# iammadab/zk

Hardware: AMD Instinct MI355X
Metric: field-ops/sec (MLE fold, 2^24 evals, BN254 Fr) + sumcheck prover wall-clock (higher is better)
Workload: dtype u256 (8 x u32 Montgomery limbs, integer)

## Files before the change

### zk_amd/csrc/capi.hip

```cpp
#include <hip/hip_runtime.h>
#include <sched.h>

#include <algorithm>
#include <array>
#include <atomic>
#include <chrono>
#include <condition_variable>
#include <mutex>
#include <cstdio>
#include <map>
#include <new>
#include <set>
#include <string>
#include <thread>
#include <utility>
#include <vector>

#include "../../include/zk_amd.h"
#include "host_core.hpp"
#include "copy_helpers.hpp"
#include "prover_state.hpp"
#include "env.hpp"
#include "kernels.cuh"
#include "eval_kernels.cuh"
// ... 763 lines not shown
    uint32_t pos = tile_log;
    for (uint32_t p = 0; p < n_pass; ++p) {
        const uint32_t L = rem / n_pass + (p < rem % n_pass ? 1u : 0u);
        k_zeta_tile<<<(uint32_t)(1ull << (n_vars - kZetaTileLog)), kBlock, kZetaLdsBytes, c->stream>>>(t->d, pos, L, c->fi->P);
        HIPCHK(hipGetLastError());
        pos += L;
    }
    return ZK_OK;
}
static int32_t coeff_to_evaluation_device_sort(zk_ctx *c, uint64_t n_vars, const uint64_t *keys, const uint64_t *coeffs, uint64_t n_terms, zk_mle **out) {
    MleHolder t;
    ZKCHK(mle_alloc(c, n_vars, t.put()));
    size_t temp_bytes = 0;
    if (zeta_sort_terms(c->stream, nullptr, n_terms, (uint32_t)n_vars, nullptr, nullptr, nullptr, nullptr, nullptr, &temp_bytes) != 0) return ZK_ERR_HIP;
    const size_t w8 = (size_t)n_terms * 8, w4 = ((size_t)n_terms * 4 + 7) & ~(size_t)7;
    PoolBlock block;
    ZKCHK(block.alloc(c, 3 * w8 + 4 * w8 + 2 * w4 + ((temp_bytes + 255) & ~(size_t)255) + 256));
    DrainOnExit drain(c);
    uint8_t *blk = block.as<uint8_t>();
    uint64_t *d_keys = reinterpret_cast<uint64_t *>(blk), *d_idx_u = d_keys + n_terms, *d_idx_s = d_idx_u + n_terms, *d_coeffs = d_idx_s + n_terms;
    uint32_t *d_pos_u = reinterpret_cast<uint32_t *>(blk + 7 * w8), *d_perm = reinterpret_cast<uint32_t *>(blk + 7 * w8 + w4);
    void *temp = blk + 7 * w8 + 2 * w4;
    HIPCHK(hipMemcpyAsync(d_keys, keys, w8, hipMemcpyHostToDevice, c->stream));
    HIPCHK(hipMemcpyAsync(d_coeffs, coeffs, 4 * w8, hipMemcpyHostToDevice, c->stream));
    if (zeta_sort_terms(c->stream, d_keys, n_terms, (uint32_t)n_vars, d_idx_u, d_pos_u, d_idx_s, d_perm, temp, &temp_bytes) != 0) return ZK_ERR_HIP;
    ZKCHK(zeta_tiled_passes(c, t.get(), n_vars, d_idx_s, d_coeffs, n_terms, d_perm));
    ZKCHK(drain.wait());
    *out = t.release();
    return ZK_OK;
}
static int32_t coeff_to_evaluation_impl(zk_ctx *c, uint64_t n_vars, const uint64_t *keys, const uint64_t *coeffs, uint64_t n_terms,
                                        zk_mle **out) {
    if (!c || !out || (n_terms && (!keys || !coeffs))) return ZK_ERR_BAD_ARG;
    if (n_vars == 0 || n_vars > kMaxVars) return ZK_ERR_EVAL_LEN;
    for (uint64_t t = 0; t < n_terms; ++t)
        if (keys[t] >> n_vars) return ZK_ERR_COEFF_RANGE;
    ZKCHK(use_device(c));
    static const bool global_passes_flag = env_flag("ZK_ZETA_GLOBAL");
    if (!global_passes_flag && n_terms && n_terms >= zeta_device_sort_min() && n_terms < ((uint64_t)1 << 32))
        return coeff_to_evaluation_device_sort(c, n_vars, keys, coeffs, n_terms, out);
    std::vector<std::pair<uint64_t, uint64_t>> order(n_terms);
    for (uint64_t t = 0; t < n_terms; ++t) order[t] = {bit_reverse64(keys[t]) >> (64 - n_vars), t};
    std::sort(order.begin(), order.end());
    const size_t stage_bytes = (size_t)n_terms * 40;
    std::vector<uint64_t> pageable;
    uint64_t *hs = nullptr;
    if (stage_bytes <= ((size_t)1 << 20)) {
        uint8_t *blk = nullptr;
        ZKCHK(results_staging(c, stage_bytes ? stage_bytes : 8, &blk));
        hs = reinterpret_cast<uint64_t *>(blk);
    } else {
        pageable.resize((size_t)n_terms * 5);
        hs = pageable.data();
    }
    uint64_t m = 0;
    {
        uint64_t *hk = hs, *hc = hs + n_terms;
        for (uint64_t i = 0; i < n_terms;) {
            Fe acc = fe_from_u64limbs(coeffs + 4 * order[i].second);
            uint64_t j = i + 1;
            for (; j < n_terms && order[j].first == order[i].first; ++j)
                acc = fe_add(acc, fe_from_u64limbs(coeffs + 4 * order[j].second), c->fi->P);
            hk[m] = order[i].first;
            fe_to_u64limbs(acc, hc + 4 * m);
            ++m;
            i = j;
        }
    }
    MleHolder t;
    ZKCHK(mle_alloc(c, n_vars, t.put()));
    PoolBlock terms;
    uint64_t *d_keys = nullptr, *d_coeffs = nullptr;
    if (m) ZKCHK(terms.alloc(c, stage_bytes));
    DrainOnExit drain(c);
    if (m) {
        HIPCHK(hipMemcpyAsync(terms.p, hs, (size_t)(n_terms + 4 * m) * 8, hipMemcpyHostToDevice, c->stream));
        d_keys = terms.as();
        d_coeffs = d_keys + n_terms;
    }
    static const bool global_passes = env_flag("ZK_ZETA_GLOBAL");
    if (!global_passes) {
        ZKCHK(zeta_tiled_passes(c, t.get(), n_vars, d_keys, d_coeffs, m, nullptr));
    } else {
        HIPCHK(hipMemsetAsync(t->d, 0, (size_t)32 << n_vars, c->stream));
        if (m) {
            k_scatter_terms<<<grid_for(m), kBlock, 0, c->stream>>>(d_keys, d_coeffs, m, t->d);
            HIPCHK(hipGetLastError());
        }
        for (uint32_t b = 0; b < n_vars;) {
            const uint32_t v = n_vars - b >= 3 ? 3u : (uint32_t)(n_vars - b);
            const uint64_t groups = 1ull << (n_vars - v);
            uint64_t g = (groups + kBlock - 1) / kBlock;
            if (g > kMaxGridStream) g = kMaxGridStream;
            if (v == 3) k_zeta_multi<3><<<(uint32_t)g, kBlock, 0, c->stream>>>(t->d, groups, b, c->fi->P);
            else if (v == 2) k_zeta_multi<2><<<(uint32_t)g, kBlock, 0, c->stream>>>(t->d, groups, b, c->fi->P);
            else k_zeta_pass<<<(uint32_t)g, kBlock, 0, c->stream>>>(t->d, groups, b, c->fi->P);
            HIPCHK(hipGetLastError());
            b += v;
        }
    }
    ZKCHK(drain.wait());
    *out = t.release();
    return ZK_OK;
}
extern "C" int32_t zk_coeff_to_evaluation(zk_ctx *c, uint64_t n_vars, const uint64_t *keys, const uint64_t *coeffs, uint64_t n_terms,
                                          zk_mle **out) {
    try {
        return coeff_to_evaluation_impl(c, n_vars, keys, coeffs, n_terms, out);
    } catch (const std::bad_alloc &) {
        return ZK_ERR_ALLOC;
    } catch (...) {
        return ZK_ERR_BAD_ARG;
    }
}

extern "C" int32_t zk_product_check(const zk_mle *const *f, uint64_t k) {
    if (k == 0) return ZK_ERR_EMPTY_PRODUCT;
    if (!f) return ZK_ERR_BAD_ARG;
    for (uint64_t i = 0; i < k; ++i) {
        if (!f[i]) return ZK_ERR_BAD_ARG;
        if (f[i]->n_vars != f[0]->n_vars) return ZK_ERR_ARITY_MISMATCH;
        if (f[i]->ctx != f[0]->ctx) return ZK_ERR_CONTEXT_MISMATCH;
    }
    return ZK_OK;
}
static int32_t product_args(zk_ctx *c, const zk_mle *const *f, uint64_t k) {
    if (!c) return ZK_ERR_BAD_ARG;
    ZKCHK(zk_product_check(f, k));
    if (f[0]->ctx != c) return ZK_ERR_CONTEXT_MISMATCH;
    if (k > (uint64_t)kMaxFactors) return ZK_ERR_UNSUPPORTED;
    return use_device(c);
}

extern "C" int32_t zk_prod_reduce(zk_ctx *c, const zk_mle *const *f, uint64_t k, zk_mle **out) {
    if (!out) return ZK_ERR_BAD_ARG;
    ZKCHK(product_args(c, f, k));
    zk_mle *o = nullptr;
    ZKCHK(mle_alloc(c, f[0]->n_vars, &o));
    FactorPtrs fp = {};
    for (uint64_t i = 0; i < k; ++i) fp.in[i] = f[i]->d;
    const uint64_t n = 1ull << f[0]->n_vars;
    if (n >= 64) {
        uint64_t g = n / kBlock;
        if (g > 2 * kMaxGridStream) g = 2 * kMaxGridStream;
        k_prod_reduce_run<<<(uint32_t)(g ? g : 1), kBlock, 0, c->stream>>>(fp, (int)k, n, o->d, c->fi->P);
    } else {
        k_prod_reduce<<<grid_for(n), kBlock, 0, c->stream>>>(fp, (int)k, n, o->d, c->fi->P);
    }
    HIPCHK(hipGetLastError());
    *out = o;
    return ZK_OK;
}

extern "C" int32_t zk_product_evaluate(zk_ctx *c, const zk_mle *const *f, uint64_t k, const uint64_t *point,
                                       uint64_t n_point, uint64_t out[4]) {
    if (!out || (!point && n_point)) return ZK_ERR_BAD_ARG;
    ZKCHK(product_args(c, f, k));
    if (n_point != f[0]->n_vars) return ZK_ERR_EVAL_ARITY;
    Fe prod = fe_one(c->fi->P);
    for (uint64_t i = 0; i < k; ++i) {
        uint64_t v[4];
        ZKCHK(zk_mle_evaluate(c, f[i], point, n_point, v));
        prod = fe_mul(prod, fe_from_u64limbs(v), c->fi->P);
    }
    fe_to_u64limbs(prod, out);
    return ZK_OK;
}

static inline uint64_t *epart_counters(uint64_t *d_epart) { return d_epart + 2 * (kEpartBytes / 8); }
static int32_t scratch_alloc(zk_ctx *c, ProverScratch &ps, uint64_t rounds, uint32_t D, const DeviceChain *chain = nullptr) {
    ps = ProverScratch{};
    ps.rp_bytes = (size_t)(rounds ? rounds : 1) * (D + 1) * 32;
    ps.ch_bytes = (size_t)(rounds ? rounds : 1) * 32;
    if (chain) {
        ps.external = true;
        ps.d_sponge = chain->d_sponge;
        ps.d_rp = chain->d_rp;
        ps.d_ch = chain->d_ch;
        ps.d_final = chain->d_final;
        ps.d_epart = chain->d_epart;
    } else {
        ZKCHK(ps.sponge_block.alloc(c, sizeof(WordSponge)));
        ps.d_sponge = ps.sponge_block.as<WordSponge>();
    }
    ZKCHK(ps.chal_block.alloc(c, kChalBlockBytes));
    ps.d_challenge = ps.chal_block.as();
    ps.d_claim = ps.d_challenge + 2 * kChalWords;
    if (chain) return ZK_OK;
    ZKCHK(ps.epart_block.alloc(c, kEpartBlockBytes));
    ps.d_epart = ps.epart_block.as();
    ZKCHK(ps.proof_block.alloc(c, ps.proof_block_bytes()));
    ps.d_rp = ps.proof_block.as();
    ps.d_ch = ps.d_rp + ps.rp_bytes / 8;
    ps.d_final = ps.d_ch + ps.ch_bytes / 8;
    return ZK_OK;
}
int32_t zk::results_staging(zk_ctx *c, size_t bytes, uint8_t **out) {
    if (c->h_results_bytes < bytes) {
        if (c->h_results) (void)hipHostFree(c->h_results);
        c->h_results = nullptr;
        c->h_results_bytes = 0;
        size_t cap = 1 << 16;
        while (cap < bytes) cap <<= 1;
        HIPCHK(hipHostMalloc((void **)&c->h_results, cap, kPolledHostFlags));
        c->h_results_bytes = cap;
    }
    *out = c->h_results;
    return ZK_OK;
}

static inline uint64_t partials_capacity() { return g_batch ? (uint64_t)kMaxGrid * kMaxSums / kMaxBatch : (uint64_t)kMaxGrid * kMaxSums; }
static inline uint64_t *partials_of(zk_ctx *c) { return g_batch ? c->d_partials + (size_t)g_batch->cur * partials_capacity() * 4 : c->d_partials; }
static inline RoundLaunchCtx launch_ctx(zk_ctx *c) {
    RoundLaunchCtx lc = {c->stream, &c->fi->P, partials_of(c), partials_capacity(), {}};
    return lc;
}
static int32_t launch_tail(zk_ctx *c, uint32_t nblocks, uint32_t ns, WordSponge *sponge, uint64_t *out_rp, uint64_t *out_ch, uint64_t *d_challenge,
                           uint64_t *lanes, const TailDerive &dv, const PendingSponge *init = nullptr) {
    const uint64_t *part = partials_of(c);
    hipStream_t st = c->stream;
    const FieldParams *P = &c->fi->P;
    if (init && init->valid && sponge == init->dst && !lanes && !g_batch) {
        k_round_tail_init<<<1, kBlock, 0, st>>>(part, nblocks, ns, sponge, out_rp, out_ch, d_challenge, *P, dv, init->w, init->zero2);
        HIPCHK(hipGetLastError());
        return ZK_OK;
    }
    if (init && init->valid) {
        k_store_sponge<<<1, 64, 0, st>>>(init->w, init->dst, init->zero2);
        HIPCHK(hipGetLastError());
    }
    auto single = [=]() {
        k_round_tail<<<1, kBlock, 0, st>>>(part, nblocks, ns, sponge, out_rp, out_ch, d_challenge, lanes, *P, dv);
        return hipGetLastError();
    };
    if (!lanes && batch_record(BK_TAIL, 0, 1, kBlock, 0, nblocks, ns, 0, 0, TailSlot{part, sponge, out_rp, out_ch, d_challenge, dv}, single)) return ZK_OK;
    HIPCHK(single());
    return ZK_OK;
}
int32_t zk::launch_reduce_tail(zk_ctx *c, uint32_t nblocks, uint32_t ns, uint64_t *out_rp) {
    k_round_tail<<<1, kBlock, 0, c->stream>>>(c->d_partials, nblocks, ns, nullptr, out_rp, nullptr, nullptr, nullptr, c->fi->P);
    HIPCHK(hipGetLastError());
    return ZK_OK;
}
static bool claim_in_round() {
    static const bool v = env_u64("ZK_CLAIM_IN_ROUND", 1, 0, 1) != 0;
    return v;
}
static inline bool fast_degree(uint32_t D) { return D >= 1 && D <= 4; }

struct TailTargets {
    WordSponge *sponge;
    uint64_t *out_rp;
    uint64_t *out_ch;
    uint64_t *d_challenge;
    uint64_t *lanes;
    const PendingSponge *init;
    uint64_t *claim_park;
    TailDerive *lanes_dv;
};
static std::vector<Fe> interp_weights_compute(uint32_t D, const FieldParams &P) {
    std::vector<Fe> w(D + 1);
    for (uint32_t i = 0; i <= D; ++i) {
        Fe den = fe_one(P);
        const Fe xi = fe_from_u32(i, P);
        for (uint32_t j = 0; j <= D; ++j)
            if (j != i) den = fe_mul(den, fe_sub(xi, fe_from_u32(j, P), P), P);
        w[i] = fe_inverse(den, P);
    }
    return w;
}
static std::vector<Fe> interp_weights(uint32_t D, const FieldParams &P) {
    static std::mutex mu;
    static std::map<std::pair<std::array<uint32_t, 8>, uint32_t>, std::vector<Fe>> cache;
    std::array<uint32_t, 8> key;
    for (int i = 0; i < 8; ++i) key[i] = P.p[i];
    std::lock_guard<std::mutex> lock(mu);
    auto it = cache.find({key, D});
    if (it == cache.end()) it = cache.emplace(std::make_pair(key, D), interp_weights_compute(D, P)).first;
    return it->second;
}
static uint64_t skip1_min_pairs() {
    static const uint64_t v = env_u64("ZK_SKIP1_MIN_PAIRS", (uint64_t)1 << 16, 1, (uint64_t)1 << 40);
    return v;
}
static inline TermSpec single_term(int k) {
    TermSpec ts = {1, {k, 0, 0, 0}};
    return ts;
}
struct DeferredTail {
    uint32_t blocks;
    bool skip1;
    bool lead;
    const uint64_t *claim;
};
static uint64_t lead_min_pairs() {
    static const uint64_t v = env_u64("ZK_LEAD_MIN_PAIRS", (uint64_t)1 << 16, 1, (uint64_t)1 << 40);
    return v;
}
static bool shard_skip_on() {
    static const bool v = env_u64("ZK_SHARD_SKIP1", 1, 0, 1) != 0;
    return v;
}
static int32_t launch_sums(zk_ctx *c, const FactorPtrs &fp, const TermSpec &ts, uint64_t q, uint32_t D, bool fused,
                           const uint64_t *d_r, const TailTargets &tt, const TailDerive *dv = nullptr, DeferredTail *defer = nullptr) {
    if (defer) defer->blocks = 0;
    const FieldParams &P = c->fi->P;
    if (fast_degree(D)) {
        uint32_t total = 0;
        int first = 0;
        const bool may_derive = !tt.lanes || (tt.lanes_dv && shard_skip_on());
        bool skip1 = dv && dv->prev_rp && tt.claim_park && fused && may_derive && D <= (uint32_t)kMaxSkipDegree && q >= skip1_min_pairs();
        bool lead = may_derive && q >= lead_min_pairs();
        ClaimJob cjob = {};
        if (skip1 && claim_in_round()) cjob = ClaimJob{dv->prev_rp, dv->prev_chal, dv->w, tt.claim_park, D + 1};
        auto with_claim = [&](RoundLaunchCtx lc) {
            lc.claim = cjob;
            return lc;
        };
        auto tail_dv = [&]() {
            TailDerive t = skip1 && dv ? *dv : TailDerive{};
            t.lead = lead ? D : 0;
            t.claim = (t.prev_rp && cjob.out) ? cjob.out : nullptr;
            if (tt.lanes) {
                if (tt.lanes_dv) *tt.lanes_dv = t;
                t.local_only = 1;
            }
            return t;
        };
        if (tt.lanes_dv) *tt.lanes_dv = TailDerive{};
        if (ts.n_terms == 2 && ts.term_k[1] == 1) {
            uint32_t g = 0;
            const int lrc = launch_round_plus1(with_claim(launch_ctx(c)), fp, ts.term_k[0], q, D, fused, d_r, &g, &skip1, &lead);
            if (lrc == kLaunchHipError) {
                g_hip_err = "round kernel launch failed";
                return ZK_ERR_HIP;
            }
            if (lrc == kLaunchOk) {
                if (defer) {
                    defer->blocks = g;
                    defer->skip1 = skip1;
                    defer->claim = skip1 ? cjob.out : nullptr;
                    defer->lead = lead;
                    return ZK_OK;
                }
                return launch_tail(c, g, D + 1, tt.sponge, tt.out_rp, tt.out_ch, tt.d_challenge, tt.lanes, tail_dv(), tt.init);
            }
        }
        if (ts.n_terms != 1) {
            skip1 = lead = false;
            cjob = {};
        }
        for (int i = 0; i < ts.n_terms; ++i) {
            FactorPtrs sub = {};
            for (int f = 0; f < ts.term_k[i]; ++f) {
                sub.in[f] = fp.in[first + f];
                sub.out[f] = fp.out[first + f];
            }
            RoundLaunchCtx lc = with_claim(launch_ctx(c));
            lc.d_partials += (size_t)total * (D + 1) * 4;
            lc.capacity_elems -= (uint64_t)total * (D + 1);
            uint32_t g = 0;
            const int lrc = launch_round(lc, sub, ts.term_k[i], q, D, fused, d_r, &g, &skip1, &lead);
            if (lrc == kLaunchUnsupported) return ZK_ERR_UNSUPPORTED;
            if (lrc != kLaunchOk) {
                g_hip_err = "round kernel launch failed";
                return ZK_ERR_HIP;
            }
            total += g;
            first += ts.term_k[i];
        }
        if (defer) {
            defer->blocks = total;
            defer->skip1 = skip1;
            defer->claim = skip1 ? cjob.out : nullptr;
            defer->lead = lead;
            return ZK_OK;
        }
        return launch_tail(c, total, D + 1, tt.sponge, tt.out_rp, tt.out_ch, tt.d_challenge, tt.lanes, tail_dv(), tt.init);
    }
    if (ts.n_terms != 1) return ZK_ERR_UNSUPPORTED;
    const int k = ts.term_k[0];
    for (uint32_t t = 0; t <= D; ++t) {
        uint32_t g = 0;
        if (launch_round_single_t(launch_ctx(c), fp, k, q, fe_from_u32(t, P), &g) != kLaunchOk) {
            g_hip_err = "round kernel launch failed";
            return ZK_ERR_HIP;
        }
        k_round_tail<<<1, kBlock, 0, c->stream>>>(c->d_partials, g, 1, nullptr, c->d_sums + 4 * t, nullptr, nullptr, nullptr, P);
        HIPCHK(hipGetLastError());
    }
    k_round_tail<<<1, kBlock, 0, c->stream>>>(c->d_sums, 1, D + 1, tt.sponge, tt.out_rp, tt.out_ch, tt.d_challenge, tt.lanes, P);
    HIPCHK(hipGetLastError());
    return ZK_OK;
}

extern "C" int32_t zk_round_sums(zk_ctx *c, const zk_mle *const *f, uint64_t k, uint32_t D, uint64_t *out) {
    if (!out) return ZK_ERR_BAD_ARG;
    ZKCHK(product_args(c, f, k));
    if (D >= kMaxSums) return ZK_ERR_UNSUPPORTED;
    if (f[0]->n_vars == 0) return ZK_ERR_PANIC_INDEX;
    FactorPtrs fp = {};
    for (uint64_t i = 0; i < k; ++i) fp.in[i] = f[i]->d;
    const uint64_t q = 1ull << (f[0]->n_vars - 1);
    uint64_t *d_out = c->d_sums + 4 * kMaxSums;
    TailTargets tt = {nullptr, d_out, nullptr, nullptr, nullptr, nullptr, nullptr};
    ZKCHK(launch_sums(c, fp, single_term((int)k), q, D, false, nullptr, tt));
    HIPCHK(hipMemcpyAsync(out, d_out, (size_t)(D + 1) * 32, hipMemcpyDeviceToHost, c->stream));
    HIPCHK(hipStreamSynchronize(c->stream));
    return ZK_OK;
}

extern "C" int32_t zk_transcript_new(zk_transcript **out) {
    if (!out) return ZK_ERR_BAD_ARG;
    zk_transcript *t = new (std::nothrow) zk_transcript();
    if (!t) return ZK_ERR_ALLOC;
    t->sp.init();
    *out = t;
    return ZK_OK;
}
extern "C" int32_t zk_transcript_free(zk_transcript *t) {
    delete t;
    return ZK_OK;
}
extern "C" int32_t zk_transcript_append(zk_transcript *t, const uint8_t *data, size_t len) {
    if (!t || (!data && len)) return ZK_ERR_BAD_ARG;
    t->sp.update(data, len);
    return ZK_OK;
}
extern "C" int32_t zk_transcript_sample_challenge(zk_transcript *t, uint8_t out[32]) {
    if (!t || !out) return ZK_ERR_BAD_ARG;
    t->sp.sample_challenge(out);
    return ZK_OK;
}
extern "C" int32_t zk_transcript_sample_field_element(zk_transcript *t, int32_t field, uint64_t out[4]) {
    if (!t || !out) return ZK_ERR_BAD_ARG;
    const FieldInfo *fi = field_info(field);
    if (!fi) return ZK_ERR_BAD_FIELD;
    uint8_t h[32];
    t->sp.sample_challenge(h);
    fe_to_u64limbs(fe_from_be_bytes_mod_order(h, 32, fi->P), out);
    return ZK_OK;
}
extern "C" int32_t zk_transcript_sample_n_field_elements(zk_transcript *t, int32_t field, uint64_t n, uint64_t *out) {
    if (!t || (!out && n)) return ZK_ERR_BAD_ARG;
    if (!field_info(field)) return ZK_ERR_BAD_FIELD;
    for (uint64_t i = 0; i < n; ++i) ZKCHK(zk_transcript_sample_field_element(t, field, out + 4 * i));
    return ZK_OK;
}
extern "C" int32_t zk_keccak256(const uint8_t *data, size_t len, uint8_t out[32]) {
    if ((!data && len) || !out) return ZK_ERR_BAD_ARG;
    Sponge s;
    s.init();
    s.update(data, len);
    s.finalize_reset(out);
    return ZK_OK;
}

void zk::absorb_elements(Sponge &sp, const uint64_t *elems, uint64_t n, const FieldParams &P) {
    uint8_t b[32];
    for (uint64_t i = 0; i < n; ++i) {
        fe_to_bytes_be(fe_from_u64limbs(elems + 4 * i), P, b);
        sp.update(b, 32);
    }
}
Fe zk::squeeze_field_element(Sponge &sp, const FieldParams &P) {
    uint8_t h[32];
    sp.sample_challenge(h);
    return fe_from_be_bytes_mod_order(h, 32, P);
}
int32_t zk::host_staging(zk_ctx *c, size_t cb) {
    if (c->h_absorb_bytes < cb) {
        for (int b = 0; b < 2; ++b) {
            if (c->h_absorb[b]) (void)hipHostFree(c->h_absorb[b]);
            c->h_absorb[b] = nullptr;
        }
        c->h_absorb_bytes = 0;
        for (int b = 0; b < 2; ++b) HIPCHK(hipHostMalloc((void **)&c->h_absorb[b], cb, hipHostMallocDefault));
        c->h_absorb_bytes = cb;
    }
    if (!c->ev_absorb[0])
        for (int b = 0; b < 2; ++b) HIPCHK(hipEventCreateWithFlags(&c->ev_absorb[b], hipEventDisableTiming));
    return ZK_OK;
}
int32_t zk::stream_table_bytes(zk_ctx *c, const zk_mle *const *f, uint64_t k, const std::function<void(const uint8_t *, size_t)> &consume) {
    const uint64_t n = 1ull << f[0]->n_vars;
    const uint64_t chunk = n < (1ull << 19) ? n : (1ull << 19);
    const size_t cb = (size_t)chunk * 32;
    const uint64_t per_table = n / chunk, total = per_table * k;
    ZKCHK(host_staging(c, cb));
    PoolBlock d_bytes[2];
    ZKCHK(d_bytes[0].alloc(c, cb));
    ZKCHK(d_bytes[1].alloc(c, cb));
    DrainOnExit drain(c);
    auto enqueue = [&](uint64_t i) -> int32_t {
        const int b = (int)(i & 1);
        const uint64_t *src = f[i / per_table]->d + 4 * (i % per_table) * chunk;
        k_to_bytes<<<grid_for(chunk), kBlock, 0, c->stream>>>(src, d_bytes[b].as<uint8_t>(), chunk, c->fi->P);
        HIPCHK(hipGetLastError());
        HIPCHK(hipMemcpyAsync(c->h_absorb[b], d_bytes[b].p, cb, hipMemcpyDeviceToHost, c->stream));
        HIPCHK(hipEventRecord(c->ev_absorb[b], c->stream));
        return ZK_OK;
    };
    ZKCHK(enqueue(0));
    for (uint64_t i = 0; i < total; ++i) {
        if (i + 1 < total) ZKCHK(enqueue(i + 1));
        HIPCHK(hipEventSynchronize(c->ev_absorb[i & 1]));
        consume(c->h_absorb[i & 1], cb);
    }
    drain.armed = false;
    return ZK_OK;
}
static int32_t absorb_tables(zk_ctx *c, Sponge &sp, zk_mle *const *f, uint64_t k) {
    return stream_table_bytes(c, (const zk_mle *const *)f, k, [&](const uint8_t *p, size_t bytes) { sp.update(p, bytes); });
}

static inline uint64_t *chal_of_round(const RoundState &st, uint64_t round) { return st.ps.d_challenge + (round & 1) * kChalWords; }
static inline uint64_t *chal_cur(const RoundState &st) { return chal_of_round(st, st.round); }
static inline uint64_t *chal_prev(const RoundState &st) { return chal_of_round(st, st.round + 1); }
static inline uint64_t *epart_of_round(const RoundState &st, uint64_t round) { return st.ps.d_epart + (round & 1) * (kEpartBytes / 8); }
static inline uint32_t *epart_counter(const RoundState &st, uint64_t round) {
    return reinterpret_cast<uint32_t *>(st.ps.d_epart + 2 * (kEpartBytes / 8) + (round & 1));
}
static int32_t round_state_init(RoundState &st, zk_ctx *c, zk_mle *const *f, uint64_t k, uint32_t D, bool consume,
                                uint64_t total_rounds, const DeviceChain *chain = nullptr) {
    st.c = c;
    st.k = k;
    st.vars_left = f[0]->n_vars;
    st.round = 0;
    st.D = D;
    st.pending_fold = false;
    st.first_out_of_place = !consume;
    st.terms = single_term((int)k);
    st.d_final = nullptr;
    st.dv = {};
    st.pipe_active = false;
    st.pipe_blocks = 0;
    st.pipe_total = true;
    st.pub = {};
    st.published = false;
    st.init.valid = false;
    for (uint64_t i = 0; i < (uint64_t)kMaxFactors; ++i) {
        st.cur[i] = i < k ? f[i]->d : nullptr;
        st.scratch[i].reset();
    }
    ZKCHK(scratch_alloc(c, st.ps, total_rounds, D, chain));
    if (D >= 1 && D <= (uint32_t)kMaxSkipDegree) {
        auto it = c->lagrange_w.find(D);
        if (it == c->lagrange_w.end()) {
            const std::vector<Fe> w = interp_weights(D, c->fi->P);
            std::vector<uint64_t> limbs(4 * (size_t)(D + 1));
            for (uint32_t t = 0; t <= D; ++t) fe_to_u64limbs(w[t], limbs.data() + 4 * t);
            RawBlock d_w;
            ZKCHK(raw_alloc(c, limbs.size() * 8, d_w.put()));
            HIPCHK(hipMemcpy(d_w.get(), limbs.data(), limbs.size() * 8, hipMemcpyHostToDevice));
            it = c->lagrange_w.emplace(D, static_cast<uint64_t *>(d_w.release())).first;
        }
        st.dv.w = it->second;
    }
    if (!consume && st.vars_left >= 2)
        for (uint64_t i = 0; i < k; ++i) ZKCHK(st.scratch[i].alloc(c, (size_t)32 << (st.vars_left - 1)));
    return ZK_OK;
}
static int32_t flush_pending_sponge(RoundState &st) {
    if (!st.init.valid) return ZK_OK;
    st.init.valid = false;
    k_store_sponge<<<1, 64, 0, st.c->stream>>>(st.init.w, st.init.dst, st.init.zero2);
    HIPCHK(hipGetLastError());
    return ZK_OK;
}
static int32_t round_enqueue(RoundState &st, uint64_t *lanes, DeferredTail *defer = nullptr, TailDerive *lanes_dv = nullptr) {
    zk_ctx *c = st.c;
    if (st.pending_fold) st.vars_left -= 1;
    const uint64_t m = st.vars_left;
    if (m == 0) return ZK_ERR_BAD_ARG;
    const uint64_t q = 1ull << (m - 1);
    FactorPtrs fp = {};
    for (uint64_t i = 0; i < st.k; ++i) {
        fp.in[i] = st.cur[i];
        fp.out[i] = (st.pending_fold && st.first_out_of_place && st.scratch[i]) ? st.scratch[i].as() : st.cur[i];
    }
    TailTargets tt;
    tt.sponge = lanes ? nullptr : st.ps.d_sponge;
    tt.out_rp = st.ps.d_rp + st.round * (st.D + 1) * 4;
    tt.out_ch = st.ps.d_ch + st.round * 4;
    tt.d_challenge = chal_cur(st);
    tt.lanes = lanes;
    tt.claim_park = st.ps.d_claim;
    tt.lanes_dv = lanes_dv;
    tt.init = nullptr;
    if (st.init.valid) {
        if (!lanes && !defer && fast_degree(st.D) && !st.pending_fold) tt.init = &st.init;
        else ZKCHK(flush_pending_sponge(st));
    }
    int32_t rc;
    if (st.pending_fold && !fast_degree(st.D)) {
        Fe r;
        (void)r;
        for (uint64_t i = 0; i < st.k; ++i) {
            k_fold_dev<<<grid_for(q * 2), kBlock, 0, c->stream>>>(fp.in[i], fp.out[i], q * 2, (uint32_t)m, c->fi->P, chal_prev(st));
            HIPCHK(hipGetLastError());
        }
        FactorPtrs g = {};
        for (uint64_t i = 0; i < st.k; ++i) g.in[i] = fp.out[i];
        rc = launch_sums(c, g, st.terms, q, st.D, false, nullptr, tt);
    } else {
        st.dv.prev_rp = st.round ? tt.out_rp - (size_t)(st.D + 1) * 4 : nullptr;
        st.dv.prev_chal = chal_prev(st);
        rc = launch_sums(c, fp, st.terms, q, st.D, st.pending_fold, chal_prev(st), tt, &st.dv, defer);
        if (tt.init) st.init.valid = false;
    }
    if (st.pending_fold) {
        for (uint64_t i = 0; i < st.k; ++i) st.cur[i] = fp.out[i];
        st.first_out_of_place = false;
    }
    st.pending_fold = true;
    return rc;
}

static uint64_t pipe_max_pairs() {
    static const uint64_t v = [] {
        uint64_t x = env_u64("ZK_PIPE_MAX_PAIRS", (uint64_t)1 << 12, 0, (uint64_t)1 << 40);
        const uint64_t cap = (uint64_t)kPipeMaxWorkBlocks * 16 * kMaxLazy;
        return x > cap ? cap : x;
    }();
    return v;
}
static inline uint64_t pipe_limit_pairs() { return pipe_max_pairs(); }
static bool pipe_shape(const RoundState &st, int *k, int *extra) {
    if (st.terms.n_terms == 1) {
        *k = st.terms.term_k[0];
        *extra = 0;
    } else if (st.terms.n_terms == 2 && st.terms.term_k[1] == 1) {
        *k = st.terms.term_k[0];
        *extra = 1;
    } else {
        return false;
    }
    return pipe_shape_ok(*k, st.D, *extra);
}
static constexpr size_t kDbgWords = 64 * 32 + 64 * 16;
static uint64_t *pipe_dbg_slot(zk_ctx *c, bool finisher) {
    static const bool on = env_flag("ZK_PIPE_DEBUG");
    if (!on) return nullptr;
    if (!c->d_dbg) {
        if (hipMalloc(&c->d_dbg, kDbgWords * 8) != hipSuccess) return nullptr;
        (void)hipMemset(c->d_dbg, 0, kDbgWords * 8);
    }
    if (finisher) return c->d_dbg + 64 * 32;
    const uint32_t i = c->dbg_launch++ % 64;
    return c->d_dbg + (size_t)i * 32;
}
static void pipe_dbg_dump(zk_ctx *c) {
    if (!c->d_dbg) return;
    std::vector<uint64_t> h(kDbgWords);
    if (hipMemcpy(h.data(), c->d_dbg, kDbgWords * 8, hipMemcpyDeviceToHost) != hipSuccess) return;
    uint64_t t0 = 0;
    for (uint32_t i = 0; i < c->dbg_launch && i < 64; ++i) {
        const uint64_t *d = h.data() + (size_t)i * 32;
        if (!t0) t0 = d[0];
        fprintf(stderr, "[pipe %2u] tail: start %7.2f red %5.2f eval %5.2f transcript %5.2f publish %5.2f | work: start %7.2f loop %5.2f close %5.2f store %5.2f\n", i,
                (d[0] - t0) / 100.0, (d[1] - d[0]) / 100.0, (d[2] - d[1]) / 100.0, (d[3] - d[2]) / 100.0, (d[4] - d[3]) / 100.0,
                d[8] ? (d[8] - t0) / 100.0 : 0.0, (d[9] - d[8]) / 100.0, (d[10] - d[9]) / 100.0, (d[11] - d[10]) / 100.0);
    }
    const uint64_t *f = h.data() + 64 * 32;
    for (uint32_t r = 0; r < 24 && f[16 * r]; ++r) {
        const uint64_t *d = f + 16 * r;
        fprintf(stderr, "[fin %2u] start %7.2f gather %5.2f eval %5.2f transcript %5.2f barrier %5.2f | work %5.2f (from %5.2f)\n", r, (d[0] - t0) / 100.0,
                (d[1] - d[0]) / 100.0, (d[2] - d[1]) / 100.0, (d[3] - d[2]) / 100.0, (d[4] - d[3]) / 100.0, d[8] ? (d[9] - d[8]) / 100.0 : 0.0,
                d[8] ? (d[8] - d[0]) / 100.0 : 0.0);
    }
    (void)hipMemset(c->d_dbg, 0, kDbgWords * 8);
    c->dbg_launch = 0;
}
static bool finish_pipe_on() {
    static const bool v = env_u64("ZK_FINISH_PIPE", 1, 0, 1) != 0;
    return v;
}
static bool finish_pipe_applies(const RoundState &st) {
    int k, extra;
    if (!finish_pipe_on() || !pipe_shape(st, &k, &extra)) return false;
    return st.vars_left >= 3 && st.vars_left - 1 <= (uint64_t)finish_pipe_max_vars(k + extra);
}
static bool pipe_wants_next(const RoundState &st, uint64_t m_s) {
    int k, extra;
    if (!pipe_limit_pairs() || !pipe_shape(st, &k, &extra)) return false;
    if (m_s < 3) return false;
    if (!finish_pipe_on() && m_s - 1 <= (uint64_t)kFinishVars) return false;
    return ((uint64_t)1 << (m_s - 2)) <= pipe_limit_pairs();
}
static int32_t finish_pipe_enqueue(RoundState &st) {
    zk_ctx *c = st.c;
    int k = 0, extra = 0;
    (void)pipe_shape(st, &k, &extra);
    FinishPipeLaunch fl = {};
    fl.k = k;
    fl.extra = extra;
    fl.D = st.D;
    fl.m_in = (uint32_t)st.vars_left;
    fl.entry = st.pipe_active ? 2 : (st.pending_fold ? 1 : 0);
    fl.e_partials = epart_of_round(st, st.round);
    fl.e_blocks = 1;
    if (st.pipe_active && !st.pipe_total) {
        fl.e_partials += (size_t)pipe_values_per_block(k, st.D) * 4;
        fl.e_blocks = st.pipe_blocks;
    }
    fl.pc = c->pipe_consts;
    fl.chal_in = chal_prev(st);
    const uint64_t remaining = st.pending_fold ? st.vars_left - 1 : st.vars_left;
    fl.chal_last = chal_of_round(st, st.round + remaining - 1);
    fl.sponge = st.ps.d_sponge;
    fl.out_rp = st.ps.d_rp + st.round * (st.D + 1) * 4;
    fl.out_ch = st.ps.d_ch + st.round * 4;
    fl.out_final = st.d_final;
    fl.dbg = pipe_dbg_slot(c, true);
    fl.pub = st.pub;
    FactorPtrs fp = {};
    for (uint64_t i = 0; i < st.k; ++i) fp.in[i] = st.cur[i];
    const int lrc = launch_finish_pipe(launch_ctx(c), fp, fl);
    if (lrc != kLaunchOk) {
        g_hip_err = "pipelined finisher launch failed";
        return lrc == kLaunchUnsupported ? ZK_ERR_UNSUPPORTED : ZK_ERR_HIP;
    }
    st.round += remaining;
    st.vars_left = 0;
    st.pending_fold = false;
    st.pipe_active = false;
    st.published = st.pub.flag != nullptr;
    return ZK_OK;
}
static PipeTailArgs pipe_tail_args(const RoundState &st, int mode, const uint64_t *partials, uint32_t nblocks, uint32_t n_in) {
    PipeTailArgs ta = {};
    ta.dbg = pipe_dbg_slot(st.c, false);
    ta.partials = partials;
    ta.nblocks = nblocks;
    ta.n_in = n_in;
    ta.mode = mode;
    ta.chal_in = chal_prev(st);
    ta.chal_out = chal_cur(st);
    ta.sponge = st.ps.d_sponge;
    ta.out_rp = st.ps.d_rp + st.round * (st.D + 1) * 4;
    ta.out_ch = st.ps.d_ch + st.round * 4;
    ta.pc = st.c->pipe_consts;
    return ta;
}
static int32_t pipe_enter(RoundState &st, const DeferredTail &dt) {
    zk_ctx *c = st.c;
    int k = 0, extra = 0;
    (void)pipe_shape(st, &k, &extra);
    PipeLaunch pl = {};
    pl.k = k;
    pl.extra = extra;
    pl.D = st.D;
    pl.fold = false;
    pl.emit = 1;
    pl.q = (uint64_t)1 << (st.vars_left - 2);
    pl.chal_fold = nullptr;
    pl.e_partials = epart_of_round(st, st.round + 1);
    pl.done_counter = epart_counter(st, st.round + 1);
    pl.tail = pipe_tail_args(st, 0, partials_of(c), dt.blocks, st.D + 1);
    if (dt.skip1) {
        pl.tail.dv = st.dv;
        pl.tail.dv.prev_rp = pl.tail.out_rp - (size_t)(st.D + 1) * 4;
        pl.tail.dv.prev_chal = chal_prev(st);
        pl.tail.dv.claim = dt.claim;
    }
    pl.tail.dv.lead = dt.lead ? st.D : 0;
    FactorPtrs fp = {};
    for (uint64_t i = 0; i < st.k; ++i) fp.in[i] = fp.out[i] = st.cur[i];
    uint32_t g = 0;
    const int lrc = launch_round_pipe(launch_ctx(c), fp, pl, &g);
    if (lrc != kLaunchOk) {
        g_hip_err = "pipelined round launch failed";
        return lrc == kLaunchUnsupported ? ZK_ERR_UNSUPPORTED : ZK_ERR_HIP;
    }
    st.pipe_active = true;
    st.pipe_blocks = g;
    st.pipe_total = true;
    return ZK_OK;
}
static int32_t pipe_step(RoundState &st) {
    zk_ctx *c = st.c;
    int k = 0, extra = 0;
    (void)pipe_shape(st, &k, &extra);
    const uint64_t m = st.vars_left;
    const bool stay = pipe_wants_next(st, m - 1);
    PipeLaunch pl = {};
    pl.k = k;
    pl.extra = extra;
    pl.D = st.D;
    pl.fold = true;
    pl.emit = stay ? 1 : 0;
    pl.q = m >= 3 ? (uint64_t)1 << (m - 3) : 0;
    if (pl.q == 0) return ZK_ERR_BAD_ARG;
    pl.chal_fold = chal_prev(st);
    pl.e_partials = epart_of_round(st, st.round + 1);
    pl.done_counter = epart_counter(st, st.round + 1);
    pl.tail = pipe_tail_args(st, 1, epart_of_round(st, st.round), 1, pipe_values_per_block(k, st.D));
    if (!st.pipe_total) {
        pl.tail.partials = epart_of_round(st, st.round) + (size_t)pipe_values_per_block(k, st.D) * 4;
        pl.tail.nblocks = st.pipe_blocks;
    }
    FactorPtrs fp = {};
    for (uint64_t i = 0; i < st.k; ++i) {
        fp.in[i] = st.cur[i];
        fp.out[i] = (st.first_out_of_place && st.scratch[i]) ? st.scratch[i].as() : st.cur[i];
    }
    uint32_t g = 0;
    const int lrc = launch_round_pipe(launch_ctx(c), fp, pl, &g);
    if (lrc != kLaunchOk) {
        g_hip_err = "pipelined round launch failed";
        return lrc == kLaunchUnsupported ? ZK_ERR_UNSUPPORTED : ZK_ERR_HIP;
    }
    for (uint64_t i = 0; i < st.k; ++i) st.cur[i] = fp.out[i];
    st.first_out_of_place = false;
    st.vars_left = m - 1;
    st.pipe_active = stay;
    st.pipe_blocks = g;
    st.pipe_total = true;
    ++st.round;
    return ZK_OK;
}

template <int K, int D>
static int32_t launch_finish(zk_ctx *c, const FactorPtrs &fp, uint32_t m_in, int pending, uint64_t *d_challenge, WordSponge *sp,
                             uint64_t *out_rp, uint64_t *out_ch, uint64_t *out_final) {
    const uint32_t m = pending ? m_in - 1 : m_in;
    const size_t lds = (size_t)K * ((size_t)32 << m) + (kBlock / 64) * (D + 1) * 32 + (D + 1) * 32 + 48;
    HIPCHK(hipFuncSetAttribute(reinterpret_cast<const void *>(&k_finish<K, D>), hipFuncAttributeMaxDynamicSharedMemorySize, (int)lds));
    hipStream_t st = c->stream;
    const FieldParams *P = &c->fi->P;
    auto single = [=]() {
        k_finish<K, D><<<1, kBlock, lds, st>>>(fp, m_in, pending, *P, d_challenge, sp, out_rp, out_ch, out_final);
        return hipGetLastError();
    };
    if (batch_record_other(single)) return ZK_OK;
    HIPCHK(single());
    return ZK_OK;
}
static bool finish_shape_ok(uint64_t k, uint32_t D) {
    const int shape = (int)k * 10 + (int)D;
    return shape == 11 || shape == 12 || shape == 21 || shape == 22 || shape == 23 || shape == 32 || shape == 33;
}
static int32_t finish_enqueue(RoundState &st) {
    zk_ctx *c = st.c;
    FactorPtrs fp = {};
    for (uint64_t i = 0; i < st.k; ++i) fp.in[i] = st.cur[i];
    const int pending = st.pending_fold ? 1 : 0;
    const uint32_t m_in = (uint32_t)st.vars_left;
    const uint64_t remaining = pending ? st.vars_left - 1 : st.vars_left;
    uint64_t *out_rp = st.ps.d_rp + st.round * (st.D + 1) * 4, *out_ch = st.ps.d_ch + st.round * 4;
    int32_t rc = ZK_ERR_UNSUPPORTED;
    if (st.terms.n_terms > 1) {
        const uint32_t m = pending ? m_in - 1 : m_in;
        const size_t lds = (size_t)st.k * ((size_t)32 << m) + (kBlock / 64) * (st.D + 1) * 32 + (st.D + 1) * 32 + 48;
        const FieldParams &P = c->fi->P;
#define ZK_FINISH_TERMS(DD)                                                                                                     \
    case DD:                                                                                                                    \
        if (hipFuncSetAttribute(reinterpret_cast<const void *>(&k_finish_terms<DD>), hipFuncAttributeMaxDynamicSharedMemorySize, \
                                (int)lds) != hipSuccess)                                                                        \
            return ZK_ERR_HIP;                                                                                                  \
        k_finish_terms<DD><<<1, kBlock, lds, c->stream>>>(fp, st.terms, m_in, pending, P, chal_prev(st), st.ps.d_sponge,     \
                                                          out_rp, out_ch, st.d_final);                                          \
        break;
        switch (st.D) {
            ZK_FINISH_TERMS(1)
            ZK_FINISH_TERMS(2)
            ZK_FINISH_TERMS(3)
            ZK_FINISH_TERMS(4)
            default: return ZK_ERR_UNSUPPORTED;
        }
#undef ZK_FINISH_TERMS
        rc = hipGetLastError() == hipSuccess ? ZK_OK : ZK_ERR_HIP;
    } else {
        switch ((int)st.k * 10 + (int)st.D) {
            case 11: rc = launch_finish<1, 1>(c, fp, m_in, pending, chal_prev(st), st.ps.d_sponge, out_rp, out_ch, st.d_final); break;
            case 12: rc = launch_finish<1, 2>(c, fp, m_in, pending, chal_prev(st), st.ps.d_sponge, out_rp, out_ch, st.d_final); break;
            case 21: rc = launch_finish<2, 1>(c, fp, m_in, pending, chal_prev(st), st.ps.d_sponge, out_rp, out_ch, st.d_final); break;
            case 22: rc = launch_finish<2, 2>(c, fp, m_in, pending, chal_prev(st), st.ps.d_sponge, out_rp, out_ch, st.d_final); break;
            case 23: rc = launch_finish<2, 3>(c, fp, m_in, pending, chal_prev(st), st.ps.d_sponge, out_rp, out_ch, st.d_final); break;
            case 32: rc = launch_finish<3, 2>(c, fp, m_in, pending, chal_prev(st), st.ps.d_sponge, out_rp, out_ch, st.d_final); break;
            case 33: rc = launch_finish<3, 3>(c, fp, m_in, pending, chal_prev(st), st.ps.d_sponge, out_rp, out_ch, st.d_final); break;
            default: break;
        }
    }
    if (rc == ZK_OK) {
        st.round += remaining;
        st.vars_left = 0;
        st.pending_fold = false;
    }
    return rc;
}
static inline bool finish_applies(const RoundState &st) {
    if (st.terms.n_terms == 1 ? !finish_shape_ok(st.k, st.D) : !fast_degree(st.D)) return false;
    const uint64_t after = st.pending_fold ? st.vars_left - 1 : st.vars_left;
    return after >= 1 && after <= (uint64_t)kFinishVars;
}

static int32_t prover_step(RoundState &st, bool *finished_in_kernel) {
    if (st.init.valid && (finish_pipe_applies(st) || st.pipe_active || finish_applies(st))) ZKCHK(flush_pending_sponge(st));
    if (finish_pipe_applies(st)) {
        *finished_in_kernel = true;
        return finish_pipe_enqueue(st);
    }
    if (st.pipe_active) return pipe_step(st);
    if (finish_applies(st)) {
        *finished_in_kernel = true;
        return finish_enqueue(st);
    }
    const uint64_t m_s = st.pending_fold ? st.vars_left - 1 : st.vars_left;
    DeferredTail dt = {0, false, false, nullptr};
    const bool enter = fast_degree(st.D) && pipe_wants_next(st, m_s);
// ... 752 lines not shown
```

### zk_amd/csrc/launch.hpp

```cpp
#pragma once
#include <hip/hip_runtime.h>
#include <stdint.h>

#include <cstring>
#include <functional>
#include <type_traits>
#include <vector>

#include "common.cuh"

namespace zk {

enum BatchKernel : int { BK_STORE_SPONGE = 1, BK_ROUND_KD, BK_ROUND0_DOT29, BK_ROUND_QUAD, BK_TAIL, BK_PIPE, BK_FINISH_PIPE, BK_OTHER };
struct BatchRecord {
    int kernel;
    uint32_t shape;
    uint32_t grid, block;
    size_t lds;
    uint64_t s[4];
    std::function<hipError_t()> single;
    alignas(16) unsigned char slot[384];
};
struct BatchRecorder {
    int n = 0;
    int cur = 0;
    hipStream_t stream = nullptr;
    const FieldParams *P = nullptr;
    std::vector<BatchRecord> recs[kMaxBatch];
    uint64_t merged = 0, replayed = 0;
};
extern thread_local BatchRecorder *g_batch;
template <class Slot, class F>
inline bool batch_record(int kernel, uint32_t shape, uint32_t grid, uint32_t block, size_t lds, uint64_t s0, uint64_t s1, uint64_t s2, uint64_t s3,
                         const Slot &slot, F &&single) {
    BatchRecorder *r = g_batch;
    if (!r) return false;
    static_assert(sizeof(Slot) <= sizeof(BatchRecord::slot), "slot does not fit a batch record");
    static_assert(std::is_trivially_copyable<Slot>::value, "slots are plain data");
    r->recs[r->cur].emplace_back();
    BatchRecord &rec = r->recs[r->cur].back();
    rec.kernel = kernel;
    rec.shape = shape;
    rec.grid = grid;
    rec.block = block;
    rec.lds = lds;
    rec.s[0] = s0, rec.s[1] = s1, rec.s[2] = s2, rec.s[3] = s3;
    rec.single = std::function<hipError_t()>(std::forward<F>(single));
    std::memcpy(rec.slot, &slot, sizeof(Slot));
    return true;
}
template <class F>
inline bool batch_record_other(F &&single) {
    struct Nothing {
        int x;
    } none = {0};
    return batch_record(BK_OTHER, 0, 0, 0, 0, 0, 0, 0, 0, none, std::forward<F>(single));
}
int batch_launch_rounds(const BatchRecorder &r, size_t idx);
int batch_launch_pipe(const BatchRecorder &r, size_t idx);
template <class Slot>
inline void batch_gather(const BatchRecorder &r, size_t idx, BatchOf<Slot> &out) {
    std::memset(&out, 0, sizeof out);
    for (int b = 0; b < r.n; ++b) std::memcpy(&out.a[b], r.recs[b][idx].slot, sizeof(Slot));
}

struct RoundLaunchCtx {
    hipStream_t stream;
    const FieldParams *P;
    uint64_t *d_partials;
    uint64_t capacity_elems;
    ClaimJob claim;
};
enum { kLaunchOk = 0, kLaunchUnsupported = -1, kLaunchHipError = -2 };
int launch_round(const RoundLaunchCtx &lc, const FactorPtrs &fp, int k, uint64_t q, uint32_t D, bool fused,
                 const uint64_t *d_r, uint32_t *out_grid, bool *skip1 = nullptr, bool *lead = nullptr);
int launch_round_plus1(const RoundLaunchCtx &lc, const FactorPtrs &fp, int k, uint64_t q, uint32_t D, bool fused,
                       const uint64_t *d_r, uint32_t *out_grid, bool *skip1 = nullptr, bool *lead = nullptr);
int launch_round_single_t(const RoundLaunchCtx &lc, const FactorPtrs &fp, int k, uint64_t q, const Fe &tval, uint32_t *out_grid);


constexpr uint32_t kPipeMaxWorkBlocks = 256;
}
#include "pipe_args.hpp"
namespace zk {
struct PipeLaunch {
    int k, extra;
    uint32_t D;
    bool fold;
    int emit;
    uint64_t q;
    const uint64_t *chal_fold;
    uint64_t *e_partials;
    uint32_t *done_counter;
    PipeTailArgs tail;
};
bool pipe_shape_ok(int k, uint32_t D, int extra);
uint32_t pipe_values_per_block(int k, uint32_t D);
uint32_t pipe_rows_per_block(int k, uint32_t D, int extra);
uint32_t pipe_work_blocks(int k, uint32_t D, int extra, uint64_t q);
int launch_round_pipe(const RoundLaunchCtx &lc, const FactorPtrs &fp, const PipeLaunch &pl, uint32_t *out_work_blocks);
int launch_spin_us(hipStream_t stream, uint32_t us);
struct FinishPipeLaunch {
    int k, extra;
    uint32_t D;
    uint32_t m_in;
    int entry;
    const uint64_t *e_partials;
    uint32_t e_blocks;
    PipeConsts pc;
    const uint64_t *chal_in;
    uint64_t *chal_last;
    WordSponge *sponge;
    uint64_t *out_rp, *out_ch, *out_final;
    uint64_t *dbg;
    FinishPublish pub;
};
int launch_finish_pipe(const RoundLaunchCtx &lc, const FactorPtrs &fp, const FinishPipeLaunch &fl);
uint32_t finish_pipe_max_vars(int n_factors);

}
```

### zk_amd/csrc/prover_state.hpp

```cpp
#pragma once
#include "host_core.hpp"

constexpr size_t kChalWords = kChallengeBytes / 8;
constexpr size_t kEpartBytes = (size_t)(kPipeMaxWorkBlocks + 2) * 16 * 32;
constexpr size_t kChalBlockBytes = 2 * kChallengeBytes + 32;
constexpr size_t kEpartBlockBytes = 2 * kEpartBytes + 16;
struct ProverScratch {
    WordSponge *d_sponge;
    uint64_t *d_challenge;
    uint64_t *d_claim;
    uint64_t *d_epart;
    uint64_t *d_rp;
    uint64_t *d_ch;
    uint64_t *d_final;
    size_t rp_bytes, ch_bytes;
    bool external;
    PoolBlock sponge_block, chal_block, epart_block, proof_block;
    size_t proof_block_bytes() const { return rp_bytes + ch_bytes + kMaxFactors * 32; }
};
struct DeviceChain {
    WordSponge *d_sponge;
    uint64_t *d_rp, *d_ch, *d_final;
    uint64_t *d_epart;
};
struct PendingSponge {
    WordSponge w;
    WordSponge *dst;
    uint64_t *zero2;
    bool valid;
};
struct RoundState {
    zk_ctx *c;
    uint64_t k;
    uint64_t vars_left;
    uint64_t round;
    uint32_t D;
    bool pending_fold;
    bool first_out_of_place;
    uint64_t *cur[kMaxFactors];
    PoolBlock scratch[kMaxFactors];
    ProverScratch ps;
    TermSpec terms;
    uint64_t *d_final;
    TailDerive dv;
    bool pipe_active;
    uint32_t pipe_blocks;
    bool pipe_total;
    PendingSponge init;
    FinishPublish pub;
    bool published;
};
struct zk_shard_prover {
    RoundState st;
    uint32_t world;
    uint64_t local_rounds, total_rounds;
    PoolBlock lanes;
    TailDerive lanes_dv;
    PoolBlock tail;
    uint32_t tail_s;
    bool tail_done;
    PoolBlock gathered;
};
```

### zk_amd/csrc/round_kernels.cuh

```cuda
#pragma once
#include "common.cuh"
#include "quad.cuh"

namespace zk {

template <int NS, bool SKIP1 = false>
ZK_D void block_reduce_store(Fe (&sum)[NS], uint64_t *__restrict__ partials, const FieldParams &P) {
    __shared__ uint32_t red[kBlock / 64][NS][8];
    const int lane = threadIdx.x & 63, wave = threadIdx.x >> 6;
#pragma unroll
    for (int t = 0; t < NS; ++t) {
        if (SKIP1 && t == 1) continue;
        sum[t] = fe_wave_sum(sum[t], P);
        if (lane == 0) {
#pragma unroll
            for (int i = 0; i < 8; ++i) red[wave][t][i] = sum[t].v[i];
        }
    }
    __syncthreads();
    if (threadIdx.x < NS && !(SKIP1 && threadIdx.x == 1)) {
        const int t = threadIdx.x;
        Fe acc;
#pragma unroll
        for (int i = 0; i < 8; ++i) acc.v[i] = red[0][t][i];
        for (int w = 1; w < kBlock / 64; ++w) {
            Fe o;
#pragma unroll
            for (int i = 0; i < 8; ++i) o.v[i] = red[w][t][i];
            acc = fe_add(acc, o, P);
        }
        fe_store(partials, (uint64_t)blockIdx.x * NS + t, acc);
    }
}

template <int D, bool FUSED>
__global__ __launch_bounds__(kBlock) void k_round(FactorPtrs fp, int k, uint64_t q, FieldParams P,
                                                  const uint64_t *__restrict__ rptr, uint64_t *__restrict__ partials) {
    constexpr int NS = D + 1;
    Mul29 r = {};
    if (FUSED) r = load_challenge29(rptr);
    Fe sum[NS];
    WideAcc acc[NS];
#pragma unroll
    for (int t = 0; t < NS; ++t) {
        sum[t] = fe_zero();
        wide_zero(acc[t]);
    }
    int lazy = 0;
    const uint64_t stride = (uint64_t)gridDim.x * kBlock;
    for (uint64_t j = (uint64_t)blockIdx.x * kBlock + threadIdx.x; j < q; j += stride) {
        Fe prod[NS];
        for (int f = 0; f < k; ++f) {
            Fe lo, hi;
            if (FUSED) {
                const Fe a0 = fe_load(fp.in[f], j), a1 = fe_load(fp.in[f], j + q);
                const Fe a2 = fe_load(fp.in[f], j + 2 * q), a3 = fe_load(fp.in[f], j + 3 * q);
                lo = fe_sub(a0, fe_mul29(fe_sub(a0, a2, P), r, P), P);
                hi = fe_sub(a1, fe_mul29(fe_sub(a1, a3, P), r, P), P);
                fe_store(fp.out[f], j, lo);
                fe_store(fp.out[f], j + q, hi);
            } else {
                lo = fe_load(fp.in[f], j);
                hi = fe_load(fp.in[f], j + q);
            }
            const Fe diff = fe_sub(hi, lo, P);
            Fe v = lo;
#pragma unroll
            for (int t = 0; t < NS; ++t) {
                if (t == 1) v = hi;
                else if (t > 1) v = fe_add(v, diff, P);
                if (k == 1) sum[t] = fe_add(sum[t], v, P);
                else if (f == 0) prod[t] = v;
                else if (f < k - 1) prod[t] = fe_mul(prod[t], v, P);
                else wide_mac(acc[t], prod[t].v, v.v);
            }
        }
        if (k > 1 && ++lazy == kMaxLazy) {
#pragma unroll
            for (int t = 0; t < NS; ++t) {
                sum[t] = fe_add(sum[t], redc_wide(acc[t], P), P);
                wide_zero(acc[t]);
            }
            lazy = 0;
        }
    }
    if (k > 1 && lazy) {
#pragma unroll
        for (int t = 0; t < NS; ++t) sum[t] = fe_add(sum[t], redc_wide(acc[t], P), P);
    }
    block_reduce_store<NS>(sum, partials, P);
}

#ifndef ZK_KD_INNER_MUL
#define ZK_KD_INNER_MUL fe_mul
#endif
template <int K, int D, bool FUSED, int EXTRA = 0>
struct RoundRegs {
    static constexpr int NS = D + 1, NL = FUSED ? 4 : 2;
    static constexpr bool DEEP = !FUSED && K + EXTRA <= 2;
    Fe cur[K + EXTRA][NL];
    Fe nxt[DEEP ? K + EXTRA : 1][DEEP ? NL : 1];
    Fe prod[NS];
    Fe sum[NS];
    Fe sum_b[EXTRA ? NS : 1];
    WideAcc acc[K > 1 ? NS : 1];
};
template <int F, int K, int D, bool FUSED, int EXTRA, bool SKIP1 = false, bool LEAD = false>
ZK_D void round_factor(RoundRegs<K, D, FUSED, EXTRA> &R, const FactorPtrs &fp, uint64_t j, uint64_t jn, bool more, uint64_t q,
                       const Mul29 &r, const FieldParams &P, uint64_t jnn = 0, bool more2 = false) {
    static_assert(!LEAD || (K == D && D >= 1), "the leading-coefficient slot needs deg = K = D");
    constexpr int NS = D + 1, NL = FUSED ? 4 : 2;
    constexpr bool PAIR3 = K == 3 && D == 3 && F == 1 && LEAD && !SKIP1;
    Fe lo, hi;
    if (FUSED) {
        lo = fe_sub(R.cur[F][0], fe_mul29(fe_sub(R.cur[F][0], R.cur[F][2], P), r, P), P);
        hi = fe_sub(R.cur[F][1], fe_mul29(fe_sub(R.cur[F][1], R.cur[F][3], P), r, P), P);
        fe_store(fp.out[F], j, lo);
        fe_store(fp.out[F], j + q, hi);
    } else {
        lo = R.cur[F][0];
        hi = R.cur[F][1];
    }
    constexpr bool DEEP = RoundRegs<K, D, FUSED, EXTRA>::DEEP;
    if (!DEEP) {
        if (more) {
#pragma unroll
            for (int l = 0; l < NL; ++l) R.cur[F][l] = fe_load(fp.in[F], jn + (uint64_t)l * q);
        }
    } else {
#pragma unroll
        for (int l = 0; l < NL; ++l) R.cur[F][l] = R.nxt[F][l];
        if (more2) {
#pragma unroll
            for (int l = 0; l < NL; ++l) R.nxt[F][l] = fe_load(fp.in[F], jnn + (uint64_t)l * q);
        }
    }
    const Fe diff = fe_sub(hi, lo, P);
    Fe v = lo;
#pragma unroll
    for (int t = 0; t < NS; ++t) {
        if (LEAD && t == D) v = diff;
        else if (t == 1) v = hi;
        else if (t > 1) v = fe_add(v, diff, P);
        if (SKIP1 && t == 1) continue;
        if (LEAD && t == D && F == K) continue;
        if (F == K) R.sum_b[t] = fe_add(R.sum_b[t], v, P);
        else if (K == 1) R.sum[t] = fe_add(R.sum[t], v, P);
        else if (F == 0) R.prod[t] = v;
        else if (PAIR3 && t == 2) continue;
        else if (F < K - 1) R.prod[t] = ZK_KD_INNER_MUL(R.prod[t], v, P);
        else wide_mac(R.acc[t], R.prod[t].v, v.v);
    }
    if (PAIR3) {
        const Fe bc = fe_add(R.prod[1], R.prod[3], P);
        R.prod[2] = fe_sub(fe_add(bc, bc, P), R.prod[0], P);
    }
}
#ifndef ZK_KD_MIN_BLOCKS
#define ZK_KD_MIN_BLOCKS(K, EXTRA, FUSED, SKIP1) (((K) + (EXTRA) <= 2 || ((K) == 3 && (EXTRA) == 0) || ((EXTRA) == 1 && (FUSED) && (SKIP1))) ? 2 : 1)
#endif
template <int K, int D, bool FUSED, int EXTRA = 0, bool SKIP1 = false, bool LEAD = false>
ZK_D void round_kd_body(const FactorPtrs &fp, uint64_t q, const FieldParams &P, const uint64_t *__restrict__ rptr, uint64_t *__restrict__ partials,
                        const ClaimJob &cj) {
    constexpr int NS = D + 1, NL = FUSED ? 4 : 2;
    uint32_t nblk = gridDim.x;
    if constexpr (SKIP1) {
        if (cj.out) {
            nblk -= 1;
            if (blockIdx.x == nblk) {
                if (threadIdx.x < 64) {
                    const Fe claim = claim_eval(cj, P);
                    if (threadIdx.x == 0) fe_store(cj.out, 0, claim);
                }
                return;
            }
        }
    }
    Mul29 r = {};
    if (FUSED) r = load_challenge29(rptr);
    RoundRegs<K, D, FUSED, EXTRA> R;
#pragma unroll
    for (int t = 0; t < NS; ++t) {
        R.sum[t] = fe_zero();
        if (EXTRA) R.sum_b[t] = fe_zero();
        if (K > 1) wide_zero(R.acc[t]);
    }
    const uint64_t stride = (uint64_t)nblk * kBlock;
    uint64_t j = (uint64_t)blockIdx.x * kBlock + threadIdx.x;
    if (j < q) {
#pragma unroll
        for (int f = 0; f < K + EXTRA; ++f)
#pragma unroll
            for (int l = 0; l < NL; ++l) R.cur[f][l] = fe_load(fp.in[f], j + (uint64_t)l * q);
    }
    if (RoundRegs<K, D, FUSED, EXTRA>::DEEP && j + stride < q) {
#pragma unroll
        for (int f = 0; f < K + EXTRA; ++f)
#pragma unroll
            for (int l = 0; l < NL; ++l) R.nxt[f][l] = fe_load(fp.in[f], j + stride + (uint64_t)l * q);
    }
    while (j < q) {
        const uint64_t jn = j + stride, jnn = jn + stride;
        const bool more = jn < q, more2 = jnn < q;
        round_factor<0, K, D, FUSED, EXTRA, SKIP1, LEAD>(R, fp, j, jn, more, q, r, P, jnn, more2);
        if constexpr (K + EXTRA > 1) round_factor<1, K, D, FUSED, EXTRA, SKIP1, LEAD>(R, fp, j, jn, more, q, r, P, jnn, more2);
        if constexpr (K + EXTRA > 2) round_factor<2, K, D, FUSED, EXTRA, SKIP1, LEAD>(R, fp, j, jn, more, q, r, P, jnn, more2);
        if constexpr (K + EXTRA > 3) round_factor<3, K, D, FUSED, EXTRA, SKIP1, LEAD>(R, fp, j, jn, more, q, r, P, jnn, more2);
        j = jn;
    }
    if (K > 1) {
#pragma unroll
        for (int t = 0; t < NS; ++t)
            if (!(SKIP1 && t == 1)) R.sum[t] = redc_wide(R.acc[t], P);
    }
    if (EXTRA) {
#pragma unroll
        for (int t = 0; t < NS; ++t)
            if (!(SKIP1 && t == 1)) R.sum[t] = fe_add(R.sum[t], R.sum_b[t], P);
    }
    block_reduce_store<NS, SKIP1>(R.sum, partials, P);
}
template <int K, int D, bool FUSED, int EXTRA = 0, bool SKIP1 = false, bool LEAD = false>
__global__ __launch_bounds__(kBlock, ZK_KD_MIN_BLOCKS(K, EXTRA, FUSED, SKIP1)) void k_round_kd(FactorPtrs fp, uint64_t q, FieldParams P,
                                                        const uint64_t *__restrict__ rptr, uint64_t *__restrict__ partials, ClaimJob cj = {}) {
    round_kd_body<K, D, FUSED, EXTRA, SKIP1, LEAD>(fp, q, P, rptr, partials, cj);
}
struct RoundSlot {
    FactorPtrs4 fp;
    const uint64_t *rptr;
    uint64_t *partials;
    ClaimJob cj;
};
template <int K, int D, bool FUSED, int EXTRA = 0, bool SKIP1 = false, bool LEAD = false>
__global__ __launch_bounds__(kBlock, ZK_KD_MIN_BLOCKS(K, EXTRA, FUSED, SKIP1)) void k_round_kd_b(BatchOf<RoundSlot> b, uint64_t q, FieldParams P) {
    const RoundSlot &a = b.a[blockIdx.y];
    const FactorPtrs fp = factor_ptrs_of(a.fp);
    round_kd_body<K, D, FUSED, EXTRA, SKIP1, LEAD>(fp, q, P, a.rptr, a.partials, a.cj);
}

ZK_D void dot29_mac(uint64_t (&c)[17], const uint32_t (&x)[9], const uint32_t (&y)[9]) {
#if defined(__HIP_DEVICE_COMPILE__) && !defined(ZK_NO_ASM)
    asm("v_mad_u64_u32 %0, vcc, %13, %18, %0\n\t"
        "v_mad_u64_u32 %1, vcc, %13, %19, %1\n\t"
        "v_mad_u64_u32 %2, vcc, %13, %20, %2\n\t"
        "v_mad_u64_u32 %3, vcc, %13, %21, %3\n\t"
        "v_mad_u64_u32 %4, vcc, %13, %22, %4\n\t"
        "v_mad_u64_u32 %5, vcc, %13, %23, %5\n\t"
        "v_mad_u64_u32 %6, vcc, %13, %24, %6\n\t"
        "v_mad_u64_u32 %7, vcc, %13, %25, %7\n\t"
        "v_mad_u64_u32 %8, vcc, %13, %26, %8\n\t"
        "v_mad_u64_u32 %1, vcc, %14, %18, %1\n\t"
        "v_mad_u64_u32 %2, vcc, %14, %19, %2\n\t"
        "v_mad_u64_u32 %3, vcc, %14, %20, %3\n\t"
        "v_mad_u64_u32 %4, vcc, %14, %21, %4\n\t"
        "v_mad_u64_u32 %5, vcc, %14, %22, %5\n\t"
        "v_mad_u64_u32 %6, vcc, %14, %23, %6\n\t"
        "v_mad_u64_u32 %7, vcc, %14, %24, %7\n\t"
        "v_mad_u64_u32 %8, vcc, %14, %25, %8\n\t"
        "v_mad_u64_u32 %9, vcc, %14, %26, %9\n\t"
        "v_mad_u64_u32 %2, vcc, %15, %18, %2\n\t"
        "v_mad_u64_u32 %3, vcc, %15, %19, %3\n\t"
        "v_mad_u64_u32 %4, vcc, %15, %20, %4\n\t"
        "v_mad_u64_u32 %5, vcc, %15, %21, %5\n\t"
        "v_mad_u64_u32 %6, vcc, %15, %22, %6\n\t"
        "v_mad_u64_u32 %7, vcc, %15, %23, %7\n\t"
        "v_mad_u64_u32 %8, vcc, %15, %24, %8\n\t"
        "v_mad_u64_u32 %9, vcc, %15, %25, %9\n\t"
        "v_mad_u64_u32 %10, vcc, %15, %26, %10\n\t"
        "v_mad_u64_u32 %3, vcc, %16, %18, %3\n\t"
        "v_mad_u64_u32 %4, vcc, %16, %19, %4\n\t"
        "v_mad_u64_u32 %5, vcc, %16, %20, %5\n\t"
        "v_mad_u64_u32 %6, vcc, %16, %21, %6\n\t"
        "v_mad_u64_u32 %7, vcc, %16, %22, %7\n\t"
        "v_mad_u64_u32 %8, vcc, %16, %23, %8\n\t"
        "v_mad_u64_u32 %9, vcc, %16, %24, %9\n\t"
        "v_mad_u64_u32 %10, vcc, %16, %25, %10\n\t"
        "v_mad_u64_u32 %11, vcc, %16, %26, %11\n\t"
        "v_mad_u64_u32 %4, vcc, %17, %18, %4\n\t"
        "v_mad_u64_u32 %5, vcc, %17, %19, %5\n\t"
        "v_mad_u64_u32 %6, vcc, %17, %20, %6\n\t"
        "v_mad_u64_u32 %7, vcc, %17, %21, %7\n\t"
        "v_mad_u64_u32 %8, vcc, %17, %22, %8\n\t"
        "v_mad_u64_u32 %9, vcc, %17, %23, %9\n\t"
        "v_mad_u64_u32 %10, vcc, %17, %24, %10\n\t"
        "v_mad_u64_u32 %11, vcc, %17, %25, %11\n\t"
        "v_mad_u64_u32 %12, vcc, %17, %26, %12"
        : "+v"(c[0]), "+v"(c[1]), "+v"(c[2]), "+v"(c[3]), "+v"(c[4]), "+v"(c[5]), "+v"(c[6]), "+v"(c[7]), "+v"(c[8]), "+v"(c[9]), "+v"(c[10]), "+v"(c[11]), "+v"(c[12])
        : "v"(x[0]), "v"(x[1]), "v"(x[2]), "v"(x[3]), "v"(x[4]), "v"(y[0]), "v"(y[1]), "v"(y[2]), "v"(y[3]), "v"(y[4]), "v"(y[5]), "v"(y[6]), "v"(y[7]), "v"(y[8])
        : "vcc");
    asm("v_mad_u64_u32 %0, vcc, %12, %16, %0\n\t"
        "v_mad_u64_u32 %1, vcc, %12, %17, %1\n\t"
        "v_mad_u64_u32 %2, vcc, %12, %18, %2\n\t"
        "v_mad_u64_u32 %3, vcc, %12, %19, %3\n\t"
        "v_mad_u64_u32 %4, vcc, %12, %20, %4\n\t"
        "v_mad_u64_u32 %5, vcc, %12, %21, %5\n\t"
        "v_mad_u64_u32 %6, vcc, %12, %22, %6\n\t"
        "v_mad_u64_u32 %7, vcc, %12, %23, %7\n\t"
        "v_mad_u64_u32 %8, vcc, %12, %24, %8\n\t"
        "v_mad_u64_u32 %1, vcc, %13, %16, %1\n\t"
        "v_mad_u64_u32 %2, vcc, %13, %17, %2\n\t"
        "v_mad_u64_u32 %3, vcc, %13, %18, %3\n\t"
        "v_mad_u64_u32 %4, vcc, %13, %19, %4\n\t"
        "v_mad_u64_u32 %5, vcc, %13, %20, %5\n\t"
        "v_mad_u64_u32 %6, vcc, %13, %21, %6\n\t"
        "v_mad_u64_u32 %7, vcc, %13, %22, %7\n\t"
        "v_mad_u64_u32 %8, vcc, %13, %23, %8\n\t"
        "v_mad_u64_u32 %9, vcc, %13, %24, %9\n\t"
        "v_mad_u64_u32 %2, vcc, %14, %16, %2\n\t"
        "v_mad_u64_u32 %3, vcc, %14, %17, %3\n\t"
        "v_mad_u64_u32 %4, vcc, %14, %18, %4\n\t"
        "v_mad_u64_u32 %5, vcc, %14, %19, %5\n\t"
        "v_mad_u64_u32 %6, vcc, %14, %20, %6\n\t"
        "v_mad_u64_u32 %7, vcc, %14, %21, %7\n\t"
        "v_mad_u64_u32 %8, vcc, %14, %22, %8\n\t"
        "v_mad_u64_u32 %9, vcc, %14, %23, %9\n\t"
        "v_mad_u64_u32 %10, vcc, %14, %24, %10\n\t"
        "v_mad_u64_u32 %3, vcc, %15, %16, %3\n\t"
        "v_mad_u64_u32 %4, vcc, %15, %17, %4\n\t"
        "v_mad_u64_u32 %5, vcc, %15, %18, %5\n\t"
        "v_mad_u64_u32 %6, vcc, %15, %19, %6\n\t"
        "v_mad_u64_u32 %7, vcc, %15, %20, %7\n\t"
        "v_mad_u64_u32 %8, vcc, %15, %21, %8\n\t"
        "v_mad_u64_u32 %9, vcc, %15, %22, %9\n\t"
        "v_mad_u64_u32 %10, vcc, %15, %23, %10\n\t"
        "v_mad_u64_u32 %11, vcc, %15, %24, %11"
        : "+v"(c[5]), "+v"(c[6]), "+v"(c[7]), "+v"(c[8]), "+v"(c[9]), "+v"(c[10]), "+v"(c[11]), "+v"(c[12]), "+v"(c[13]), "+v"(c[14]), "+v"(c[15]), "+v"(c[16])
        : "v"(x[5]), "v"(x[6]), "v"(x[7]), "v"(x[8]), "v"(y[0]), "v"(y[1]), "v"(y[2]), "v"(y[3]), "v"(y[4]), "v"(y[5]), "v"(y[6]), "v"(y[7]), "v"(y[8])
        : "vcc");
#else
#pragma unroll
    for (int i = 0; i < 9; ++i)
#pragma unroll
        for (int j = 0; j < 9; ++j) c[i + j] += (uint64_t)x[i] * y[j];
#endif
}

ZK_D void dot29_normalise(uint64_t (&c)[17]) {
    constexpr uint64_t M = (1ull << 29) - 1;
#pragma unroll
    for (int k = 0; k < 16; ++k) {
        c[k + 1] += c[k] >> 29;
        c[k] &= M;
    }
}
ZK_D void dot29_to_wide(const uint64_t (&c)[17], WideAcc &w) {
    constexpr uint64_t M = (1ull << 29) - 1;
    uint64_t window = 0;
    int have = 0, wi = 0;
#pragma unroll
    for (int k = 0; k < 18; ++k) {
        const uint64_t limb = k < 16 ? c[k] : (k == 16 ? (c[16] & M) : (c[16] >> 29));
        window |= limb << have;
        have += 29;
        if (have >= 32) {
            if (wi < 17) w.v[wi] = (uint32_t)window;
            ++wi;
            window >>= 32;
            have -= 32;
        }
    }
    if (wi < 17) w.v[wi++] = (uint32_t)window;
#pragma unroll
    for (int i = 0; i < 17; ++i)
        if (i >= wi) w.v[i] = 0;
}
template <int EXTRA>
ZK_D void round0_dot29_body(const FactorPtrs &fp, uint64_t q, const FieldParams &P, uint64_t *__restrict__ partials) {
    constexpr int NT = 2 + EXTRA;
    uint64_t c0[17], c1[17], cL[17];
#pragma unroll
    for (int k = 0; k < 17; ++k) c0[k] = c1[k] = cL[k] = 0;
    Fe sb0 = fe_zero(), sb1 = fe_zero();
    constexpr bool DEEP = EXTRA == 0;
    Fe cur[NT][2], nxt[DEEP ? NT : 1][2];
    const uint64_t stride = (uint64_t)gridDim.x * kBlock;
    uint64_t j = (uint64_t)blockIdx.x * kBlock + threadIdx.x;
    if (j < q) {
#pragma unroll
        for (int f = 0; f < NT; ++f) cur[f][0] = fe_load(fp.in[f], j), cur[f][1] = fe_load(fp.in[f], j + q);
    }
    if (DEEP && j + stride < q) {
#pragma unroll
        for (int f = 0; f < NT; ++f) nxt[f][0] = fe_load(fp.in[f], j + stride), nxt[f][1] = fe_load(fp.in[f], j + stride + q);
    }
    int since = 0;
    while (j < q) {
        const uint64_t jn = j + stride, jnn = jn + stride;
        Fe v[NT][2];
#pragma unroll
        for (int f = 0; f < NT; ++f) v[f][0] = cur[f][0], v[f][1] = cur[f][1];
        if (DEEP) {
#pragma unroll
            for (int f = 0; f < NT; ++f) cur[f][0] = nxt[f][0], cur[f][1] = nxt[f][1];
            if (jnn < q) {
#pragma unroll
                for (int f = 0; f < NT; ++f) nxt[f][0] = fe_load(fp.in[f], jnn), nxt[f][1] = fe_load(fp.in[f], jnn + q);
            }
        } else if (jn < q) {
#pragma unroll
            for (int f = 0; f < NT; ++f) cur[f][0] = fe_load(fp.in[f], jn), cur[f][1] = fe_load(fp.in[f], jn + q);
        }
        uint32_t a[9], b[9];
        split29(v[0][0].v, a);
        split29(v[1][0].v, b);
        dot29_mac(c0, a, b);
        split29(v[0][1].v, a);
        split29(v[1][1].v, b);
        dot29_mac(c1, a, b);
        const Fe d0 = fe_sub(v[0][1], v[0][0], P), d1 = fe_sub(v[1][1], v[1][0], P);
        split29(d0.v, a);
        split29(d1.v, b);
        dot29_mac(cL, a, b);
        if (EXTRA) {
            sb0 = fe_add(sb0, v[NT - 1][0], P);
            sb1 = fe_add(sb1, v[NT - 1][1], P);
        }
        if (++since == 7) {
            dot29_normalise(c0);
            dot29_normalise(c1);
            dot29_normalise(cL);
            since = 0;
        }
        j = jn;
    }
    dot29_normalise(c0);
    dot29_normalise(c1);
    dot29_normalise(cL);
    Fe sum[3];
    {
        WideAcc w;
        dot29_to_wide(c0, w);
        sum[0] = redc_wide(w, P);
        dot29_to_wide(c1, w);
        sum[1] = redc_wide(w, P);
        dot29_to_wide(cL, w);
        sum[2] = redc_wide(w, P);
    }
    if (EXTRA) {
        sum[0] = fe_add(sum[0], sb0, P);
        sum[1] = fe_add(sum[1], sb1, P);
    }
    block_reduce_store<3>(sum, partials, P);
}
template <int EXTRA>
__global__ __launch_bounds__(kBlock, 2) void k_round0_dot29(FactorPtrs fp, uint64_t q, FieldParams P, uint64_t *__restrict__ partials) {
    round0_dot29_body<EXTRA>(fp, q, P, partials);
}
template <int EXTRA>
__global__ __launch_bounds__(kBlock, 2) void k_round0_dot29_b(BatchOf<RoundSlot> b, uint64_t q, FieldParams P) {
    const RoundSlot &a = b.a[blockIdx.y];
    const FactorPtrs fp = factor_ptrs_of(a.fp);
    round0_dot29_body<EXTRA>(fp, q, P, a.partials);
}

extern __shared__ __attribute__((aligned(1024))) uint8_t glds_ring[];
constexpr uint32_t kGldsRingBytes = 4 * 8192, kGldsRing3Bytes = 4 * 12288;
template <int N>
ZK_D void wait_vm() {
    asm volatile("s_waitcnt vmcnt(%0)" ::"n"(N) : "memory");
}
#define ZK_GLDS_PIECES(ADDR)                      \
    "global_load_lds_dwordx4 %1, " ADDR " nt\n\t" \
    "global_load_lds_dwordx4 %1, " ADDR " offset:1024 nt\n\t"
#define ZK_GLDS_ROW(M0, ADDR) "s_mov_b32 m0, " M0 "\n\ts_nop 0\n\t" ZK_GLDS_PIECES(ADDR)
ZK_D void glds_rows2(uint64_t a0, uint64_t a1, uint32_t voff, uint32_t lds_dst) {
    unsigned keep;
    asm volatile("s_mov_b32 %0, m0\n\t" ZK_GLDS_ROW("%4", "%2") ZK_GLDS_ROW("%5", "%3") "s_mov_b32 m0, %0"
                 : "=&s"(keep)
                 : "v"(voff), "s"(a0), "s"(a1), "s"(lds_dst), "s"(lds_dst + 2048u)
                 : "memory");
}
ZK_D void glds_rows4(uint64_t a0, uint64_t a1, uint64_t a2, uint64_t a3, uint32_t voff, uint32_t lds_dst) {
    unsigned keep;
    asm volatile("s_mov_b32 %0, m0\n\t" ZK_GLDS_ROW("%6", "%2") ZK_GLDS_ROW("%7", "%3") ZK_GLDS_ROW("%8", "%4") ZK_GLDS_ROW("%9", "%5") "s_mov_b32 m0, %0"
                 : "=&s"(keep)
                 : "v"(voff), "s"(a0), "s"(a1), "s"(a2), "s"(a3), "s"(lds_dst), "s"(lds_dst + 2048u), "s"(lds_dst + 4096u), "s"(lds_dst + 6144u)
                 : "memory");
}
#undef ZK_GLDS_ROW
#undef ZK_GLDS_PIECES
ZK_D Fe glds_elem(const uint8_t *row, uint32_t elem) {
    const uint4 *p = reinterpret_cast<const uint4 *>(row + elem * 32);
    const uint4 a = p[0], b = p[1];
    Fe r = {{a.x, a.y, a.z, a.w, b.x, b.y, b.z, b.w}};
    return r;
}
struct GldsWave {
    uint8_t *my;
    uint32_t my_lds;
    uint32_t lane, voff, own;
    uint64_t r0, rs, K;
};
ZK_D GldsWave glds_wave(uint64_t q, uint32_t nblk, uint32_t bytes_per_wave = 8192) {
    GldsWave w;
    w.lane = threadIdx.x & 63;
    const uint32_t wave = __builtin_amdgcn_readfirstlane(threadIdx.x >> 6);
    w.my = glds_ring + wave * bytes_per_wave;
    w.my_lds = __builtin_amdgcn_readfirstlane((uint32_t)(uintptr_t)w.my);
    w.voff = w.lane * 16;
    w.own = pair_owned(w.lane);
    const uint64_t runs = q >> 6;
    w.r0 = (uint64_t)blockIdx.x * (kBlock / 64) + wave;
    w.rs = (uint64_t)nblk * (kBlock / 64);
    w.K = w.r0 < runs ? (runs - w.r0 + w.rs - 1) / w.rs : 0;
    return w;
}

template <int NU, int F>
ZK_D void round0_glds_wait(bool last) {
    if (!last) wait_vm<4 * (NU - 1)>();
    else wait_vm<4 * (NU - 1 - F)>();
}
ZK_D void dot29_flush(uint64_t (&c)[17], Fe &sum, const FieldParams &P) {
    WideAcc wa;
    dot29_to_wide(c, wa);
    sum = fe_add(sum, redc_wide(wa, P), P);
#pragma unroll
    for (int i = 0; i < 17; ++i) c[i] = 0;
}
template <int EXTRA>
ZK_D void round0_glds_body(const FactorPtrs &fp, uint64_t q, const FieldParams &P, uint64_t *__restrict__ partials) {
    constexpr int NU = 2 + EXTRA;
    const GldsWave w = glds_wave(q, gridDim.x, NU * 4096);
    const uint64_t hi_off = q * 32;
    uint64_t c0[17], c1[17], cL[17];
#pragma unroll
    for (int k = 0; k < 17; ++k) c0[k] = c1[k] = cL[k] = 0;
    Fe sum[3] = {fe_zero(), fe_zero(), fe_zero()};
    Fe sb0 = fe_zero(), sb1 = fe_zero();
    if (w.K) {
#pragma unroll
        for (int f = 0; f < NU; ++f) {
            const uint64_t a = (uint64_t)(uintptr_t)fp.in[f] + w.r0 * 2048;
            glds_rows2(a, a + hi_off, w.voff, w.my_lds + f * 4096);
        }
        int since = 0, lazy = 0;
        for (uint64_t k = 0; k < w.K; ++k) {
            const bool last = k + 1 == w.K;
            const uint64_t next = (w.r0 + (k + 1) * w.rs) * 2048;
            uint32_t la0[9], la1[9], ld0[9];
            round0_glds_wait<NU, 0>(last);
            {
                const Fe lo = glds_elem(w.my, w.lane), hi = glds_elem(w.my + 2048, w.lane);
                asm volatile("s_waitcnt lgkmcnt(0)" ::: "memory");
                if (!last) glds_rows2((uint64_t)(uintptr_t)fp.in[0] + next, (uint64_t)(uintptr_t)fp.in[0] + next + hi_off, w.voff, w.my_lds);
                split29(lo.v, la0);
                split29(hi.v, la1);
                const Fe d = fe_sub(hi, lo, P);
                split29(d.v, ld0);
            }
            round0_glds_wait<NU, 1>(last);
            {
                const Fe lo = glds_elem(w.my + 4096, w.lane), hi = glds_elem(w.my + 6144, w.lane);
                asm volatile("s_waitcnt lgkmcnt(0)" ::: "memory");
                if (!last) glds_rows2((uint64_t)(uintptr_t)fp.in[1] + next, (uint64_t)(uintptr_t)fp.in[1] + next + hi_off, w.voff, w.my_lds + 4096);
                uint32_t b[9];
                split29(lo.v, b);
                dot29_mac(c0, la0, b);
                split29(hi.v, b);
                dot29_mac(c1, la1, b);
                const Fe d = fe_sub(hi, lo, P);
                split29(d.v, b);
                dot29_mac(cL, ld0, b);
            }
            if constexpr (EXTRA) {
                round0_glds_wait<NU, 2>(last);
                const Fe lo = glds_elem(w.my + 8192, w.lane), hi = glds_elem(w.my + 10240, w.lane);
                asm volatile("s_waitcnt lgkmcnt(0)" ::: "memory");
                if (!last) glds_rows2((uint64_t)(uintptr_t)fp.in[2] + next, (uint64_t)(uintptr_t)fp.in[2] + next + hi_off, w.voff, w.my_lds + 8192);
                sb0 = fe_add(sb0, lo, P);
                sb1 = fe_add(sb1, hi, P);
            }
            ++lazy;
            if (++since == 7 || lazy == kMaxLazy || last) {
                dot29_normalise(c0);
                dot29_normalise(c1);
                dot29_normalise(cL);
                since = 0;
            }
            if (lazy == kMaxLazy || last) {
                dot29_flush(c0, sum[0], P);
                dot29_flush(c1, sum[1], P);
                dot29_flush(cL, sum[2], P);
                lazy = 0;
            }
        }
    }
    if (EXTRA) {
        sum[0] = fe_add(sum[0], sb0, P);
        sum[1] = fe_add(sum[1], sb1, P);
    }
    block_reduce_store<3>(sum, partials, P);
}
template <int EXTRA>
__global__ __launch_bounds__(kBlock, 2) void k_round0_glds(FactorPtrs fp, uint64_t q, FieldParams P, uint64_t *__restrict__ partials) {
    round0_glds_body<EXTRA>(fp, q, P, partials);
}
template <int EXTRA>
__global__ __launch_bounds__(kBlock, 2) void k_round0_glds_b(BatchOf<RoundSlot> b, uint64_t q, FieldParams P) {
    const RoundSlot &a = b.a[blockIdx.y];
    const FactorPtrs fp = factor_ptrs_of(a.fp);
    round0_glds_body<EXTRA>(fp, q, P, a.partials);
}

template <int F, int K, int EXTRA, bool STORE_NT>
ZK_D void fused_glds_unit(const GldsWave &w, const FactorPtrs &fp, uint64_t q, uint64_t run, bool last, const Mul29 &r, const FieldParams &P,
                          Fe (&prod)[K + 1], WideAcc (&acc)[K + 1], Fe (&sum_b)[K + 1]) {
    constexpr int D = K, NT = K + EXTRA;
    const Fe c0 = glds_elem(w.my, w.own), c1 = glds_elem(w.my + 2048, w.own), c2 = glds_elem(w.my + 4096, w.own), c3 = glds_elem(w.my + 6144, w.own);
    asm volatile("s_waitcnt lgkmcnt(0)" ::: "memory");
    const uint64_t rowb = q * 32;
    if (F + 1 < NT) {
        const uint64_t a = (uint64_t)(uintptr_t)fp.in[F + 1 < NT ? F + 1 : 0] + run * 2048;
        glds_rows4(a, a + rowb, a + 2 * rowb, a + 3 * rowb, w.voff, w.my_lds);
    } else if (!last) {
        const uint64_t a = (uint64_t)(uintptr_t)fp.in[0] + (run + w.rs) * 2048;
        glds_rows4(a, a + rowb, a + 2 * rowb, a + 3 * rowb, w.voff, w.my_lds);
    }
    const Fe lo = fe_sub(c0, fe_mul29(fe_sub(c0, c2, P), r, P), P);
    const Fe hi = fe_sub(c1, fe_mul29(fe_sub(c1, c3, P), r, P), P);
    uint64_t *out = fp.out[F];
    if (STORE_NT) {
        run_store_nt(out + run * 256, w.lane, lo);
        run_store_nt(out + (run * 64 + q) * 4, w.lane, hi);
    } else {
        run_store(out + run * 256, w.lane, lo);
        run_store(out + (run * 64 + q) * 4, w.lane, hi);
    }
    const Fe diff = fe_sub(hi, lo, P);
    Fe v = lo;
#pragma unroll
    for (int t = 0; t <= D; ++t) {
        if (t == 1) {
            v = hi;
            continue;
        }
        if (t == D) v = diff;
        else if (t > 1) v = fe_add(v, diff, P);
        if (F == K) {
            if (t < D) sum_b[t] = fe_add(sum_b[t], v, P);
        } else if (F == 0) prod[t] = v;
        else if (F < K - 1) prod[t] = ZK_KD_INNER_MUL(prod[t], v, P);
        else wide_mac(acc[t], prod[t].v, v.v);
    }
    if (F + 1 < NT || !last) wait_vm<4>();
}
template <int K, int EXTRA, bool STORE_NT>
ZK_D void fused_glds_body(const FactorPtrs &fp, uint64_t q, const FieldParams &P, const uint64_t *__restrict__ rptr, uint64_t *__restrict__ partials,
                          const ClaimJob &cj) {
    constexpr int NS = K + 1;
    uint32_t nblk = gridDim.x;
    if (cj.out) {
        nblk -= 1;
        if (blockIdx.x == nblk) {
            if (threadIdx.x < 64) {
                const Fe claim = claim_eval(cj, P);
                if (threadIdx.x == 0) fe_store(cj.out, 0, claim);
            }
            return;
        }
    }
    const Mul29 r = load_challenge29(rptr);
    asm volatile("s_waitcnt vmcnt(0)" ::: "memory");
    const GldsWave w = glds_wave(q, nblk);
    Fe prod[NS], sum[NS], sum_b[NS];
    WideAcc acc[NS];
#pragma unroll
    for (int t = 0; t < NS; ++t) {
        sum[t] = fe_zero();
        sum_b[t] = fe_zero();
        wide_zero(acc[t]);
    }
    if (w.K) {
        {
            const uint64_t a = (uint64_t)(uintptr_t)fp.in[0] + w.r0 * 2048, rowb = q * 32;
            glds_rows4(a, a + rowb, a + 2 * rowb, a + 3 * rowb, w.voff, w.my_lds);
        }
        wait_vm<0>();
        for (uint64_t k = 0; k < w.K; ++k) {
            const uint64_t run = w.r0 + k * w.rs;
            const bool last = k + 1 == w.K;
            fused_glds_unit<0, K, EXTRA, STORE_NT>(w, fp, q, run, last, r, P, prod, acc, sum_b);
            fused_glds_unit<1, K, EXTRA, STORE_NT>(w, fp, q, run, last, r, P, prod, acc, sum_b);
            if constexpr (K + EXTRA > 2) fused_glds_unit<2, K, EXTRA, STORE_NT>(w, fp, q, run, last, r, P, prod, acc, sum_b);
            if constexpr (K + EXTRA > 3) fused_glds_unit<3, K, EXTRA, STORE_NT>(w, fp, q, run, last, r, P, prod, acc, sum_b);
        }
#pragma unroll
        for (int t = 0; t < NS; ++t)
            if (t != 1) sum[t] = redc_wide(acc[t], P);
        if (EXTRA) {
#pragma unroll
            for (int t = 0; t < K; ++t)
                if (t != 1) sum[t] = fe_add(sum[t], sum_b[t], P);
        }
    }
    block_reduce_store<NS, true>(sum, partials, P);
}
template <int K, int EXTRA, bool STORE_NT>
__global__ __launch_bounds__(kBlock, 2) void k_round_fused_glds(FactorPtrs fp, uint64_t q, FieldParams P, const uint64_t *__restrict__ rptr,
                                                                 uint64_t *__restrict__ partials, ClaimJob cj) {
    fused_glds_body<K, EXTRA, STORE_NT>(fp, q, P, rptr, partials, cj);
}
template <int K, int EXTRA, bool STORE_NT>
__global__ __launch_bounds__(kBlock, 2) void k_round_fused_glds_b(BatchOf<RoundSlot> b, uint64_t q, FieldParams P) {
    const RoundSlot &a = b.a[blockIdx.y];
    const FactorPtrs fp = factor_ptrs_of(a.fp);
    fused_glds_body<K, EXTRA, STORE_NT>(fp, q, P, a.rptr, a.partials, a.cj);
}

template <int K, int D, int EXTRA>
ZK_D void round_quad_body(const FactorPtrs &fp, uint64_t q, const FieldParams &P, const uint64_t *__restrict__ rptr, uint64_t *__restrict__ partials) {
    constexpr int NF = K + EXTRA, NS = D + 1;
    static_assert(NF <= 4 && NS <= 4, "four lanes per pair index");
    __shared__ uint32_t red[kBlock / 64][4][8];
    const Mul29 r = load_challenge29(rptr);
    const uint32_t lane = threadIdx.x & 63, wave = threadIdx.x >> 6, l4 = lane & 3;
    const bool has_factor = l4 < (uint32_t)NF;
    const uint64_t *in = fp.in[0];
    uint64_t *out = fp.out[0];
#pragma unroll
    for (int f = 1; f < NF; ++f)
        if (l4 == (uint32_t)f) {
            in = fp.in[f];
            out = fp.out[f];
        }
    const uint64_t stride = (uint64_t)gridDim.x * (kBlock / 4);
    uint64_t j = (uint64_t)blockIdx.x * (kBlock / 4) + (threadIdx.x >> 2);
    WideAcc acc;
    wide_zero(acc);
    Fe sum = fe_zero();
    Fe cur[4];
#pragma unroll
    for (int l = 0; l < 4; ++l) cur[l] = fe_zero();
    if (j < q && has_factor) {
#pragma unroll
        for (int l = 0; l < 4; ++l) cur[l] = fe_load(in, j + (uint64_t)l * q);
    }
    while (j < q) {
        const uint64_t jn = j + stride;
        Fe v[NS];
        v[0] = fe_sub(cur[0], fe_mul29(fe_sub(cur[0], cur[2], P), r, P), P);
        const Fe hi = fe_sub(cur[1], fe_mul29(fe_sub(cur[1], cur[3], P), r, P), P);
        if (has_factor) {
            fe_store(out, j, v[0]);
            fe_store(out, j + q, hi);
            if (jn < q) {
#pragma unroll
                for (int l = 0; l < 4; ++l) cur[l] = fe_load(in, jn + (uint64_t)l * q);
            }
        }
        if constexpr (NS > 1) v[1] = hi;
        if constexpr (NS > 2) {
            const Fe diff = fe_sub(hi, v[0], P);
#pragma unroll
            for (int t = 2; t < NS; ++t) v[t] = fe_add(v[t - 1], diff, P);
        }
        Fe w[NF];
#pragma unroll
        for (int g = 0; g < NF; ++g) w[g] = fe_zero();
        quad_transpose<0, NF, NS>(v, w, l4);
        if constexpr (K == 1) {
            sum = fe_add(sum, w[0], P);
        } else {
            Fe prod = w[0];
#pragma unroll
            for (int g = 1; g + 1 < K; ++g) prod = ZK_KD_INNER_MUL(prod, w[g], P);
            wide_mac(acc, prod.v, w[K - 1].v);
        }
        if constexpr (EXTRA) sum = fe_add(sum, w[K], P);
        j = jn;
    }
    Fe s = sum;
    if constexpr (K > 1) s = fe_add(redc_wide(acc, P), sum, P);
    {
        Fe a, b;
#pragma unroll
        for (int i = 0; i < 8; ++i) {
            const auto x = __builtin_amdgcn_permlane32_swap(s.v[i], s.v[i], false, false);
            a.v[i] = x[0];
            b.v[i] = x[1];
        }
        s = fe_add(a, b, P);
#pragma unroll
        for (int i = 0; i < 8; ++i) {
            const auto x = __builtin_amdgcn_permlane16_swap(s.v[i], s.v[i], false, false);
            a.v[i] = x[0];
            b.v[i] = x[1];
        }
        s = fe_add(a, b, P);
        s = fe_add(s, fe_dpp<0x128>(s), P);
        s = fe_add(s, fe_dpp<0x12C>(s), P);
    }
    if (lane < 4) {
#pragma unroll
        for (int i = 0; i < 8; ++i) red[wave][lane][i] = s.v[i];
    }
    __syncthreads();
    if (threadIdx.x < (uint32_t)NS) {
        Fe tot = fe_zero();
        for (int wv = 0; wv < kBlock / 64; ++wv) {
            Fe o;
#pragma unroll
            for (int i = 0; i < 8; ++i) o.v[i] = red[wv][threadIdx.x][i];
            tot = fe_add(tot, o, P);
        }
        fe_store(partials, (uint64_t)blockIdx.x * NS + threadIdx.x, tot);
    }
}
template <int K, int D, int EXTRA>
__global__ __launch_bounds__(kBlock) void k_round_quad(FactorPtrs fp, uint64_t q, FieldParams P, const uint64_t *__restrict__ rptr,
                                                       uint64_t *__restrict__ partials) {
    round_quad_body<K, D, EXTRA>(fp, q, P, rptr, partials);
}
template <int K, int D, int EXTRA>
__global__ __launch_bounds__(kBlock) void k_round_quad_b(BatchOf<RoundSlot> b, uint64_t q, FieldParams P) {
    const RoundSlot &a = b.a[blockIdx.y];
    const FactorPtrs fp = factor_ptrs_of(a.fp);
    round_quad_body<K, D, EXTRA>(fp, q, P, a.rptr, a.partials);
}

__global__ __launch_bounds__(kBlock) void k_round_single_t(FactorPtrs fp, int k, uint64_t q, FieldParams P, Fe tval,
                                                           uint64_t *__restrict__ partials) {
    Fe sum[1] = {fe_zero()};
    const uint64_t stride = (uint64_t)gridDim.x * kBlock;
    for (uint64_t j = (uint64_t)blockIdx.x * kBlock + threadIdx.x; j < q; j += stride) {
        Fe prod = fe_zero();
        for (int f = 0; f < k; ++f) {
            const Fe lo = fe_load(fp.in[f], j), hi = fe_load(fp.in[f], j + q);
            const Fe v = fe_sub(lo, fe_mul(tval, fe_sub(lo, hi, P), P), P);
            prod = (f == 0) ? v : fe_mul(prod, v, P);
        }
        sum[0] = fe_add(sum[0], prod, P);
    }
    block_reduce_store<1>(sum, partials, P);
}

}
```

### zk_amd/csrc/rounds.hip

```cpp
#include <cstdlib>

#include "env.hpp"
#include "launch.hpp"
#include "round_kernels.cuh"

namespace zk {

static constexpr uint32_t kCapGrid = 2048;

static uint32_t min_blocks() {
    static const uint32_t v = (uint32_t)env_u64("ZK_ROUND_MIN_BLOCKS", 512, 1, 2048);
    return v;
}
static int round0_dot29_mode() {
    static const int v = (int)env_u64("ZK_ROUND0_DOT29", 1, 0, 2);
    return v;
}
static bool round0_dot29() { return round0_dot29_mode() != 0; }
static bool round0_dot29_extra() { return round0_dot29_mode() == 2; }
static bool glds_rounds() {
    static const bool v = env_u64("ZK_ROUND_GLDS", 1, 0, 1) != 0;
    return v;
}
static uint64_t glds_min_pairs(uint64_t unset) {
    static const uint64_t v = env_u64("ZK_ROUND_GLDS_MIN_PAIRS", 0, 0, (uint64_t)1 << 40);
    return v ? v : unset;
}
static uint64_t glds_nt_min_pairs() {
    static const uint64_t v = env_u64("ZK_ROUND_GLDS_NT_MIN_PAIRS", (uint64_t)1 << 20, 64, (uint64_t)1 << 40);
    return v;
}
static bool glds_takes(uint64_t q, uint64_t min_pairs) { return glds_rounds() && (q & 63) == 0 && q >= 64 && q >= glds_min_pairs(min_pairs); }
static uint64_t quad_max_pairs() {
    static const uint64_t v = env_u64("ZK_QUAD_MAX_PAIRS", (uint64_t)1 << 15, 0, (uint64_t)1 << 40);
    return v;
}
template <int K, int D, int EXTRA>
static uint32_t launch_quad(const RoundLaunchCtx &lc, const FactorPtrs &fp, uint64_t q, const uint64_t *d_r) {
    uint64_t g = (q + 63) / 64;
    const uint64_t cap = (q + 64ull * kMaxLazy - 1) / (64ull * kMaxLazy);
    if (g > 2048) g = cap > 2048 ? cap : 2048;
    const FieldParams *P = lc.P;
    hipStream_t st = lc.stream;
    uint64_t *part = lc.d_partials;
    const uint32_t grid = (uint32_t)g;
    auto single = [=]() {
        k_round_quad<K, D, EXTRA><<<grid, kBlock, 0, st>>>(fp, q, *P, d_r, part);
        return hipGetLastError();
    };
    if (!batch_record(BK_ROUND_QUAD, (uint32_t)K | ((uint32_t)D << 4) | ((uint32_t)EXTRA << 9), grid, kBlock, 0, q, 0, 0, 0,
                      RoundSlot{factor_ptrs4(fp), d_r, part, ClaimJob{}}, single))
        (void)single();
    return grid;
}
static uint32_t min_blocks_plus1() {
    static const uint32_t v = (uint32_t)env_u64("ZK_ROUND_MIN_BLOCKS", 256, 1, 2048);
    return v;
}
static inline uint32_t round_grid(uint64_t q, uint32_t min_b = min_blocks()) {
    uint64_t b = (q + (uint64_t)kBlock * kMaxLazy - 1) / ((uint64_t)kBlock * kMaxLazy);
    const uint64_t one_pair = (q + kBlock - 1) / kBlock;
    const uint64_t floor_b = one_pair < min_b ? one_pair : min_b;
    if (b < floor_b) b = floor_b;
    return (uint32_t)(b ? b : 1);
}
static inline uint32_t capped_grid(uint64_t q) {
    uint64_t b = (q + kBlock - 1) / kBlock;
    if (b > kCapGrid) b = kCapGrid;
    return (uint32_t)(b ? b : 1);
}

static inline uint32_t claim_blocks(const RoundLaunchCtx &lc) { return lc.claim.out ? 1u : 0u; }

thread_local BatchRecorder *g_batch = nullptr;

constexpr uint32_t kd_shape(int K, int D, bool FUSED, int EXTRA, bool SKIP1, bool LEAD) {
    return (uint32_t)K | ((uint32_t)D << 4) | ((uint32_t)FUSED << 8) | ((uint32_t)EXTRA << 9) | ((uint32_t)SKIP1 << 10) | ((uint32_t)LEAD << 11);
}
template <int K, int D, bool FUSED, int EXTRA = 0, bool SKIP1 = false, bool LEAD = false>
static void go_kd(const RoundLaunchCtx &lc, const FactorPtrs &fp, uint64_t q, const uint64_t *d_r, uint32_t grid, const ClaimJob &cj = {}) {
    const FieldParams *P = lc.P;
    hipStream_t st = lc.stream;
    uint64_t *part = lc.d_partials;
    auto single = [=]() {
        k_round_kd<K, D, FUSED, EXTRA, SKIP1, LEAD><<<grid, kBlock, 0, st>>>(fp, q, *P, d_r, part, cj);
        return hipGetLastError();
    };
    if (batch_record(BK_ROUND_KD, kd_shape(K, D, FUSED, EXTRA, SKIP1, LEAD), grid, kBlock, 0, q, 0, 0, 0, RoundSlot{factor_ptrs4(fp), d_r, part, cj}, single))
        return;
    (void)single();
}
template <int EXTRA>
static void go_round0_dot29(const RoundLaunchCtx &lc, const FactorPtrs &fp, uint64_t q, uint32_t grid) {
    const FieldParams *P = lc.P;
    hipStream_t st = lc.stream;
    uint64_t *part = lc.d_partials;
    auto single = [=]() {
        k_round0_dot29<EXTRA><<<grid, kBlock, 0, st>>>(fp, q, *P, part);
        return hipGetLastError();
    };
    if (batch_record(BK_ROUND0_DOT29, (uint32_t)EXTRA, grid, kBlock, 0, q, 0, 0, 0, RoundSlot{factor_ptrs4(fp), nullptr, part, ClaimJob{}}, single)) return;
    (void)single();
}

constexpr uint32_t kShapeGlds = 1u << 12, kShapeGldsNt = 1u << 13;
template <int EXTRA>
static void go_round0_glds(const RoundLaunchCtx &lc, const FactorPtrs &fp, uint64_t q, uint32_t grid) {
    const FieldParams *P = lc.P;
    hipStream_t st = lc.stream;
    uint64_t *part = lc.d_partials;
    constexpr uint32_t lds = EXTRA ? kGldsRing3Bytes : kGldsRingBytes;
    auto single = [=]() {
        k_round0_glds<EXTRA><<<grid, kBlock, lds, st>>>(fp, q, *P, part);
        return hipGetLastError();
    };
    if (batch_record(BK_ROUND0_DOT29, kShapeGlds | (uint32_t)EXTRA, grid, kBlock, lds, q, 0, 0, 0, RoundSlot{factor_ptrs4(fp), nullptr, part, ClaimJob{}}, single)) return;
    (void)single();
}
template <int K, int EXTRA>
static void go_fused_glds(const RoundLaunchCtx &lc, const FactorPtrs &fp, uint64_t q, const uint64_t *d_r, uint32_t grid, const ClaimJob &cj) {
    const FieldParams *P = lc.P;
    hipStream_t st = lc.stream;
    uint64_t *part = lc.d_partials;
    const bool nt = q >= glds_nt_min_pairs();
    auto single = [=]() {
        if (nt) k_round_fused_glds<K, EXTRA, true><<<grid, kBlock, kGldsRingBytes, st>>>(fp, q, *P, d_r, part, cj);
        else k_round_fused_glds<K, EXTRA, false><<<grid, kBlock, kGldsRingBytes, st>>>(fp, q, *P, d_r, part, cj);
        return hipGetLastError();
    };
    if (batch_record(BK_ROUND_KD, kd_shape(K, K, true, EXTRA, true, true) | kShapeGlds | (nt ? kShapeGldsNt : 0u), grid, kBlock, kGldsRingBytes, q, 0, 0, 0,
                     RoundSlot{factor_ptrs4(fp), d_r, part, cj}, single))
        return;
    (void)single();
}

template <int K, int D>
static void launch_kd(const RoundLaunchCtx &lc, const FactorPtrs &fp, uint64_t q, bool fused, const uint64_t *d_r, uint32_t g) {
    if (fused) go_kd<K, D, true>(lc, fp, q, d_r, g);
    else go_kd<K, D, false>(lc, fp, q, d_r, g);
}
template <int D>
static void launch_generic(const RoundLaunchCtx &lc, const FactorPtrs &fp, int k, uint64_t q, bool fused, const uint64_t *d_r, uint32_t g) {
    const FieldParams *P = lc.P;
    hipStream_t st = lc.stream;
    uint64_t *part = lc.d_partials;
    auto single = [=]() {
        if (fused) k_round<D, true><<<g, kBlock, 0, st>>>(fp, k, q, *P, d_r, part);
        else k_round<D, false><<<g, kBlock, 0, st>>>(fp, k, q, *P, d_r, part);
        return hipGetLastError();
    };
    if (!batch_record_other(single)) (void)single();
}

int launch_round(const RoundLaunchCtx &lc, const FactorPtrs &fp, int k, uint64_t q, uint32_t D, bool fused,
                 const uint64_t *d_r, uint32_t *out_grid, bool *skip1, bool *lead) {
    if (D < 1 || D > 4 || k < 1 || k > kMaxFactors) return kLaunchUnsupported;
    uint32_t g = round_grid(q);
    bool no_lead = false;
    if (!lead) lead = &no_lead;
    if (*lead && !((k == 2 && D == 2) || (k == 3 && D == 3))) *lead = false;
    if (*lead && (uint64_t)g * (D + 1) <= lc.capacity_elems) {
        const int shl = k * 10 + (int)D;
        bool done = true;
        if (!fused) {
            if (shl == 22 && round0_dot29() && glds_takes(q, (uint64_t)1 << 21)) {
                if (g > 512) g = 512;
                go_round0_glds<0>(lc, fp, q, g);
            } else if (shl == 22 && round0_dot29()) go_round0_dot29<0>(lc, fp, q, g);
            else if (shl == 22) go_kd<2, 2, false, 0, false, true>(lc, fp, q, d_r, g);
            else go_kd<3, 3, false, 0, false, true>(lc, fp, q, d_r, g);
            if (skip1) *skip1 = false;
        } else if (skip1 && *skip1) {
            if (shl == 33 && glds_takes(q, (uint64_t)1 << 16)) go_fused_glds<3, 0>(lc, fp, q, d_r, g + claim_blocks(lc), lc.claim);
            else if (shl == 22) go_kd<2, 2, true, 0, true, true>(lc, fp, q, d_r, g + claim_blocks(lc), lc.claim);
            else go_kd<3, 3, true, 0, true, true>(lc, fp, q, d_r, g + claim_blocks(lc), lc.claim);
        } else {
            done = false;
        }
        if (done) {
            if (hipGetLastError() != hipSuccess) return kLaunchHipError;
            *out_grid = g;
            return kLaunchOk;
        }
    }
    *lead = false;
    if (fused && q >= 16 && q <= 4 * quad_max_pairs() && (uint64_t)2048 * (D + 1) <= lc.capacity_elems) {
        const int shq = k * 10 + (int)D;
        uint32_t gq = 0;
        if (shq == 22 && q <= quad_max_pairs()) gq = launch_quad<2, 2, 0>(lc, fp, q, d_r);
        else if (shq == 33) gq = launch_quad<3, 3, 0>(lc, fp, q, d_r);
        if (gq) {
            if (skip1) *skip1 = false;
            if (hipGetLastError() != hipSuccess) return kLaunchHipError;
            *out_grid = gq;
            return kLaunchOk;
        }
    }
    if (skip1 && *skip1) {
        const bool fits1 = (uint64_t)g * (D + 1) <= lc.capacity_elems;
        const int shape1 = (fits1 && fused) ? k * 10 + (int)D : 0;
        if (shape1 == 22) go_kd<2, 2, true, 0, true>(lc, fp, q, d_r, g + claim_blocks(lc), lc.claim);
        else if (shape1 == 33) go_kd<3, 3, true, 0, true>(lc, fp, q, d_r, g + claim_blocks(lc), lc.claim);
        else *skip1 = false;
        if (*skip1) {
            if (hipGetLastError() != hipSuccess) return kLaunchHipError;
            *out_grid = g;
            return kLaunchOk;
        }
    }
    const bool fits = (uint64_t)g * (D + 1) <= lc.capacity_elems;
    const int shape = fits ? k * 10 + (int)D : 0;
    switch (shape) {
        case 11: launch_kd<1, 1>(lc, fp, q, fused, d_r, g); break;
        case 12: launch_kd<1, 2>(lc, fp, q, fused, d_r, g); break;
        case 21: launch_kd<2, 1>(lc, fp, q, fused, d_r, g); break;
        case 22: launch_kd<2, 2>(lc, fp, q, fused, d_r, g); break;
        case 23: launch_kd<2, 3>(lc, fp, q, fused, d_r, g); break;
        case 32: launch_kd<3, 2>(lc, fp, q, fused, d_r, g); break;
        case 33: launch_kd<3, 3>(lc, fp, q, fused, d_r, g); break;
        default:
            g = capped_grid(q);
            switch (D) {
                case 1: launch_generic<1>(lc, fp, k, q, fused, d_r, g); break;
                case 2: launch_generic<2>(lc, fp, k, q, fused, d_r, g); break;
                case 3: launch_generic<3>(lc, fp, k, q, fused, d_r, g); break;
                default: launch_generic<4>(lc, fp, k, q, fused, d_r, g); break;
            }
    }
    if (hipGetLastError() != hipSuccess) return kLaunchHipError;
    *out_grid = g;
    return kLaunchOk;
}

int launch_round_plus1(const RoundLaunchCtx &lc, const FactorPtrs &fp, int k, uint64_t q, uint32_t D, bool fused,
                       const uint64_t *d_r, uint32_t *out_grid, bool *skip1, bool *lead) {
    uint32_t g = round_grid(q, min_blocks_plus1());
    if ((uint64_t)g * (D + 1) > lc.capacity_elems) return kLaunchUnsupported;
    const int shape = k * 10 + (int)D;
    bool no_lead = false;
    if (!lead) lead = &no_lead;
    if (*lead && shape == 22 && (!fused || (skip1 && *skip1))) {
        if (!fused) {
            if (round0_dot29_extra()) go_round0_dot29<1>(lc, fp, q, g);
            else if (round0_dot29() && glds_takes(q, (uint64_t)1 << 20)) {
                if (g > 512) g = 512;
                go_round0_glds<1>(lc, fp, q, g);
            } else go_kd<2, 2, false, 1, false, true>(lc, fp, q, d_r, g);
            if (skip1) *skip1 = false;
        } else {
            if (glds_takes(q, (uint64_t)1 << 19)) go_fused_glds<2, 1>(lc, fp, q, d_r, g + claim_blocks(lc), lc.claim);
            else go_kd<2, 2, true, 1, true, true>(lc, fp, q, d_r, g + claim_blocks(lc), lc.claim);
        }
        if (hipGetLastError() != hipSuccess) return kLaunchHipError;
        *out_grid = g;
        return kLaunchOk;
    }
    *lead = false;
    if (fused && shape == 22 && q >= 16 && q <= quad_max_pairs() && (uint64_t)2048 * (D + 1) <= lc.capacity_elems) {
        const uint32_t gq = launch_quad<2, 2, 1>(lc, fp, q, d_r);
        if (skip1) *skip1 = false;
        if (hipGetLastError() != hipSuccess) return kLaunchHipError;
        *out_grid = gq;
        return kLaunchOk;
    }
    if (skip1 && *skip1 && !(shape == 22 && fused)) *skip1 = false;
    if (shape == 22) {
        if (fused && skip1 && *skip1) go_kd<2, 2, true, 1, true>(lc, fp, q, d_r, g + claim_blocks(lc), lc.claim);
        else if (fused) go_kd<2, 2, true, 1>(lc, fp, q, d_r, g);
        else go_kd<2, 2, false, 1>(lc, fp, q, d_r, g);
    } else if (shape == 33) {
        if (fused) go_kd<3, 3, true, 1>(lc, fp, q, d_r, g);
        else go_kd<3, 3, false, 1>(lc, fp, q, d_r, g);
    } else {
        return kLaunchUnsupported;
    }
    if (hipGetLastError() != hipSuccess) return kLaunchHipError;
    *out_grid = g;
    return kLaunchOk;
}

int launch_round_single_t(const RoundLaunchCtx &lc, const FactorPtrs &fp, int k, uint64_t q, const Fe &tval, uint32_t *out_grid) {
    const uint32_t g = capped_grid(q);
    {
        const FieldParams *P = lc.P;
        hipStream_t st = lc.stream;
        uint64_t *part = lc.d_partials;
        auto single = [=]() {
            k_round_single_t<<<g, kBlock, 0, st>>>(fp, k, q, *P, tval, part);
            return hipGetLastError();
        };
        if (!batch_record_other(single)) (void)single();
    }
    if (hipGetLastError() != hipSuccess) return kLaunchHipError;
    *out_grid = g;
    return kLaunchOk;
}

int batch_launch_rounds(const BatchRecorder &r, size_t idx) {
    const BatchRecord &r0 = r.recs[0][idx];
    BatchOf<RoundSlot> slots;
    batch_gather(r, idx, slots);
    const dim3 grid(r0.grid, (uint32_t)r.n);
    const uint64_t q = r0.s[0];
    const FieldParams &P = *r.P;
#define ZK_KD_B(K, D, F, E, S, L)                                                                  \
    case kd_shape(K, D, F, E, S, L):                                                               \
        k_round_kd_b<K, D, F, E, S, L><<<grid, kBlock, 0, r.stream>>>(slots, q, P);               \
        break;
    if (r0.kernel == BK_ROUND_KD && (r0.shape & kShapeGlds)) {
        const uint32_t base = r0.shape & ~(kShapeGlds | kShapeGldsNt);
        const bool nt = (r0.shape & kShapeGldsNt) != 0;
        if (base == kd_shape(3, 3, true, 0, true, true)) {
            if (nt) k_round_fused_glds_b<3, 0, true><<<grid, kBlock, kGldsRingBytes, r.stream>>>(slots, q, P);
            else k_round_fused_glds_b<3, 0, false><<<grid, kBlock, kGldsRingBytes, r.stream>>>(slots, q, P);
        } else {
            return kLaunchUnsupported;
        }
    } else if (r0.kernel == BK_ROUND_KD) {
        switch (r0.shape) {
            ZK_KD_B(2, 2, true, 0, true, true)
            ZK_KD_B(3, 3, true, 0, true, true)
            ZK_KD_B(3, 3, false, 0, false, true)
            ZK_KD_B(2, 2, true, 0, false, false)
            ZK_KD_B(3, 3, true, 0, false, false)
            ZK_KD_B(2, 2, false, 0, false, false)
            ZK_KD_B(3, 3, false, 0, false, false)
            default: return kLaunchUnsupported;
        }
    } else if (r0.kernel == BK_ROUND0_DOT29 && r0.shape == kShapeGlds) {
        k_round0_glds_b<0><<<grid, kBlock, kGldsRingBytes, r.stream>>>(slots, q, P);
    } else if (r0.kernel == BK_ROUND0_DOT29 && r0.shape == (kShapeGlds | 1u)) {
        k_round0_glds_b<1><<<grid, kBlock, kGldsRing3Bytes, r.stream>>>(slots, q, P);
    } else if (r0.kernel == BK_ROUND0_DOT29) {
        if (r0.shape != 0) return kLaunchUnsupported;
        k_round0_dot29_b<0><<<grid, kBlock, 0, r.stream>>>(slots, q, P);
    } else if (r0.kernel == BK_ROUND_QUAD) {
        if (r0.shape == (2u | (2u << 4))) k_round_quad_b<2, 2, 0><<<grid, kBlock, 0, r.stream>>>(slots, q, P);
        else if (r0.shape == (3u | (3u << 4))) k_round_quad_b<3, 3, 0><<<grid, kBlock, 0, r.stream>>>(slots, q, P);
        else return kLaunchUnsupported;
    } else {
        return kLaunchUnsupported;
    }
#undef ZK_KD_B
    return hipGetLastError() == hipSuccess ? kLaunchOk : kLaunchHipError;
}

}
```

Measured before the change: 197.6 billion.

## Alternate sweep direction across sumcheck rounds to reuse cached tail data

Adds a per-round reverse flag that XOR-permutes the block/run index so consecutive fused round kernels traverse the MLE buffers in opposite directions. The data touched last by one round is then read first by the next, which is meant to raise hits in the last-level/infinity cache when the working set exceeds it. The flag is only enabled when the combined size of two consecutive rounds passes a byte threshold. It costs an extra XOR per index, and mismatched permutations of lo/hi halves could be a risk if q is not a power of two, though it falls back to identity in that case.

After: 197.1 billion. Within noise of the previous version (-0.2%).

```diff
diff --git a/zk_amd/csrc/capi.hip b/zk_amd/csrc/capi.hip
--- a/zk_amd/csrc/capi.hip
+++ b/zk_amd/csrc/capi.hip
@@ -1089,7 +1089,8 @@
     return v;
 }
 static int32_t launch_sums(zk_ctx *c, const FactorPtrs &fp, const TermSpec &ts, uint64_t q, uint32_t D, bool fused,
-                           const uint64_t *d_r, const TailTargets &tt, const TailDerive *dv = nullptr, DeferredTail *defer = nullptr) {
+                           const uint64_t *d_r, const TailTargets &tt, const TailDerive *dv = nullptr, DeferredTail *defer = nullptr,
+                           bool reverse = false) {
     if (defer) defer->blocks = 0;
     const FieldParams &P = c->fi->P;
     if (fast_degree(D)) {
@@ -1102,6 +1103,7 @@
         if (skip1 && claim_in_round()) cjob = ClaimJob{dv->prev_rp, dv->prev_chal, dv->w, tt.claim_park, D + 1};
         auto with_claim = [&](RoundLaunchCtx lc) {
             lc.claim = cjob;
+            lc.reverse = reverse;
             return lc;
         };
         auto tail_dv = [&]() {
@@ -1317,6 +1319,8 @@
     st.D = D;
     st.pending_fold = false;
     st.first_out_of_place = !consume;
+    st.sweep_rev = false;
+    st.sweep_bytes = 0;
     st.terms = single_term((int)k);
     st.d_final = nullptr;
     st.dv = {};
@@ -1393,7 +1397,16 @@
     } else {
         st.dv.prev_rp = st.round ? tt.out_rp - (size_t)(st.D + 1) * 4 : nullptr;
         st.dv.prev_chal = chal_prev(st);
-        rc = launch_sums(c, fp, st.terms, q, st.D, st.pending_fold, chal_prev(st), tt, &st.dv, defer);
+        bool reverse = false;
+        if (st.pending_fold) {
+            const uint64_t bytes = st.k * q * 192;
+            if (sweep_alternates(bytes, st.sweep_bytes)) reverse = !st.sweep_rev;
+            st.sweep_bytes = bytes;
+        } else {
+            st.sweep_bytes = 0;
+        }
+        st.sweep_rev = reverse;
+        rc = launch_sums(c, fp, st.terms, q, st.D, st.pending_fold, chal_prev(st), tt, &st.dv, defer, reverse);
         if (tt.init) st.init.valid = false;
     }
     if (st.pending_fold) {
diff --git a/zk_amd/csrc/launch.hpp b/zk_amd/csrc/launch.hpp
--- a/zk_amd/csrc/launch.hpp
+++ b/zk_amd/csrc/launch.hpp
@@ -70,7 +70,9 @@
     uint64_t *d_partials;
     uint64_t capacity_elems;
     ClaimJob claim;
+    bool reverse;
 };
+bool sweep_alternates(uint64_t bytes, uint64_t prev_bytes);
 enum { kLaunchOk = 0, kLaunchUnsupported = -1, kLaunchHipError = -2 };
 int launch_round(const RoundLaunchCtx &lc, const FactorPtrs &fp, int k, uint64_t q, uint32_t D, bool fused,
                  const uint64_t *d_r, uint32_t *out_grid, bool *skip1 = nullptr, bool *lead = nullptr);
diff --git a/zk_amd/csrc/prover_state.hpp b/zk_amd/csrc/prover_state.hpp
--- a/zk_amd/csrc/prover_state.hpp
+++ b/zk_amd/csrc/prover_state.hpp
@@ -49,6 +49,8 @@
     PendingSponge init;
     FinishPublish pub;
     bool published;
+    bool sweep_rev = false;
+    uint64_t sweep_bytes = 0;
 };
 struct zk_shard_prover {
     RoundState st;
diff --git a/zk_amd/csrc/round_kernels.cuh b/zk_amd/csrc/round_kernels.cuh
--- a/zk_amd/csrc/round_kernels.cuh
+++ b/zk_amd/csrc/round_kernels.cuh
@@ -1,6 +1,7 @@
 #pragma once
 #include "common.cuh"
 #include "quad.cuh"
+#include "sweep_index.hpp"
 
 namespace zk {
 
@@ -161,7 +162,7 @@
 #endif
 template <int K, int D, bool FUSED, int EXTRA = 0, bool SKIP1 = false, bool LEAD = false>
 ZK_D void round_kd_body(const FactorPtrs &fp, uint64_t q, const FieldParams &P, const uint64_t *__restrict__ rptr, uint64_t *__restrict__ partials,
-                        const ClaimJob &cj) {
+                        const ClaimJob &cj, uint64_t rev = 0) {
     constexpr int NS = D + 1, NL = FUSED ? 4 : 2;
     uint32_t nblk = gridDim.x;
     if constexpr (SKIP1) {
@@ -191,21 +192,22 @@
 #pragma unroll
         for (int f = 0; f < K + EXTRA; ++f)
 #pragma unroll
-            for (int l = 0; l < NL; ++l) R.cur[f][l] = fe_load(fp.in[f], j + (uint64_t)l * q);
+            for (int l = 0; l < NL; ++l) R.cur[f][l] = fe_load(fp.in[f], sweep_index(j, rev) + (uint64_t)l * q);
     }
     if (RoundRegs<K, D, FUSED, EXTRA>::DEEP && j + stride < q) {
 #pragma unroll
         for (int f = 0; f < K + EXTRA; ++f)
 #pragma unroll
-            for (int l = 0; l < NL; ++l) R.nxt[f][l] = fe_load(fp.in[f], j + stride + (uint64_t)l * q);
+            for (int l = 0; l < NL; ++l) R.nxt[f][l] = fe_load(fp.in[f], sweep_index(j + stride, rev) + (uint64_t)l * q);
     }
     while (j < q) {
         const uint64_t jn = j + stride, jnn = jn + stride;
         const bool more = jn < q, more2 = jnn < q;
-        round_factor<0, K, D, FUSED, EXTRA, SKIP1, LEAD>(R, fp, j, jn, more, q, r, P, jnn, more2);
-        if constexpr (K + EXTRA > 1) round_factor<1, K, D, FUSED, EXTRA, SKIP1, LEAD>(R, fp, j, jn, more, q, r, P, jnn, more2);
-        if constexpr (K + EXTRA > 2) round_factor<2, K, D, FUSED, EXTRA, SKIP1, LEAD>(R, fp, j, jn, more, q, r, P, jnn, more2);
-        if constexpr (K + EXTRA > 3) round_factor<3, K, D, FUSED, EXTRA, SKIP1, LEAD>(R, fp, j, jn, more, q, r, P, jnn, more2);
+        const uint64_t pj = sweep_index(j, rev), pjn = sweep_index(jn, rev), pjnn = sweep_index(jnn, rev);
+        round_factor<0, K, D, FUSED, EXTRA, SKIP1, LEAD>(R, fp, pj, pjn, more, q, r, P, pjnn, more2);
+        if constexpr (K + EXTRA > 1) round_factor<1, K, D, FUSED, EXTRA, SKIP1, LEAD>(R, fp, pj, pjn, more, q, r, P, pjnn, more2);
+        if constexpr (K + EXTRA > 2) round_factor<2, K, D, FUSED, EXTRA, SKIP1, LEAD>(R, fp, pj, pjn, more, q, r, P, pjnn, more2);
+        if constexpr (K + EXTRA > 3) round_factor<3, K, D, FUSED, EXTRA, SKIP1, LEAD>(R, fp, pj, pjn, more, q, r, P, pjnn, more2);
         j = jn;
     }
     if (K > 1) {
@@ -222,8 +224,9 @@
 }
 template <int K, int D, bool FUSED, int EXTRA = 0, bool SKIP1 = false, bool LEAD = false>
 __global__ __launch_bounds__(kBlock, ZK_KD_MIN_BLOCKS(K, EXTRA, FUSED, SKIP1)) void k_round_kd(FactorPtrs fp, uint64_t q, FieldParams P,
-                                                        const uint64_t *__restrict__ rptr, uint64_t *__restrict__ partials, ClaimJob cj = {}) {
-    round_kd_body<K, D, FUSED, EXTRA, SKIP1, LEAD>(fp, q, P, rptr, partials, cj);
+                                                        const uint64_t *__restrict__ rptr, uint64_t *__restrict__ partials, ClaimJob cj = {},
+                                                        uint64_t rev = 0) {
+    round_kd_body<K, D, FUSED, EXTRA, SKIP1, LEAD>(fp, q, P, rptr, partials, cj, rev);
 }
 struct RoundSlot {
     FactorPtrs4 fp;
@@ -232,10 +235,11 @@
     ClaimJob cj;
 };
 template <int K, int D, bool FUSED, int EXTRA = 0, bool SKIP1 = false, bool LEAD = false>
-__global__ __launch_bounds__(kBlock, ZK_KD_MIN_BLOCKS(K, EXTRA, FUSED, SKIP1)) void k_round_kd_b(BatchOf<RoundSlot> b, uint64_t q, FieldParams P) {
+__global__ __launch_bounds__(kBlock, ZK_KD_MIN_BLOCKS(K, EXTRA, FUSED, SKIP1)) void k_round_kd_b(BatchOf<RoundSlot> b, uint64_t q, FieldParams P,
+                                                                                                 uint64_t rev = 0) {
     const RoundSlot &a = b.a[blockIdx.y];
     const FactorPtrs fp = factor_ptrs_of(a.fp);
-    round_kd_body<K, D, FUSED, EXTRA, SKIP1, LEAD>(fp, q, P, a.rptr, a.partials, a.cj);
+    round_kd_body<K, D, FUSED, EXTRA, SKIP1, LEAD>(fp, q, P, a.rptr, a.partials, a.cj, rev);
 }
 
 ZK_D void dot29_mac(uint64_t (&c)[17], const uint32_t (&x)[9], const uint32_t (&y)[9]) {
@@ -365,7 +369,7 @@
         if (i >= wi) w.v[i] = 0;
 }
 template <int EXTRA>
-ZK_D void round0_dot29_body(const FactorPtrs &fp, uint64_t q, const FieldParams &P, uint64_t *__restrict__ partials) {
+ZK_D void round0_dot29_body(const FactorPtrs &fp, uint64_t q, const FieldParams &P, uint64_t *__restrict__ partials, uint64_t rev = 0) {
     constexpr int NT = 2 + EXTRA;
     uint64_t c0[17], c1[17], cL[17];
 #pragma unroll
@@ -377,11 +381,12 @@
     uint64_t j = (uint64_t)blockIdx.x * kBlock + threadIdx.x;
     if (j < q) {
 #pragma unroll
-        for (int f = 0; f < NT; ++f) cur[f][0] = fe_load(fp.in[f], j), cur[f][1] = fe_load(fp.in[f], j + q);
+        for (int f = 0; f < NT; ++f) cur[f][0] = fe_load(fp.in[f], sweep_index(j, rev)), cur[f][1] = fe_load(fp.in[f], sweep_index(j, rev) + q);
     }
     if (DEEP && j + stride < q) {
 #pragma unroll
-        for (int f = 0; f < NT; ++f) nxt[f][0] = fe_load(fp.in[f], j + stride), nxt[f][1] = fe_load(fp.in[f], j + stride + q);
+        for (int f = 0; f < NT; ++f)
+            nxt[f][0] = fe_load(fp.in[f], sweep_index(j + stride, rev)), nxt[f][1] = fe_load(fp.in[f], sweep_index(j + stride, rev) + q);
     }
     int since = 0;
     while (j < q) {
@@ -394,11 +399,11 @@
             for (int f = 0; f < NT; ++f) cur[f][0] = nxt[f][0], cur[f][1] = nxt[f][1];
             if (jnn < q) {
 #pragma unroll
-                for (int f = 0; f < NT; ++f) nxt[f][0] = fe_load(fp.in[f], jnn), nxt[f][1] = fe_load(fp.in[f], jnn + q);
+                for (int f = 0; f < NT; ++f) nxt[f][0] = fe_load(fp.in[f], sweep_index(jnn, rev)), nxt[f][1] = fe_load(fp.in[f], sweep_index(jnn, rev) + q);
             }
         } else if (jn < q) {
 #pragma unroll
-            for (int f = 0; f < NT; ++f) cur[f][0] = fe_load(fp.in[f], jn), cur[f][1] = fe_load(fp.in[f], jn + q);
+            for (int f = 0; f < NT; ++f) cur[f][0] = fe_load(fp.in[f], sweep_index(jn, rev)), cur[f][1] = fe_load(fp.in[f], sweep_index(jn, rev) + q);
         }
         uint32_t a[9], b[9];
         split29(v[0][0].v, a);
@@ -443,14 +448,14 @@
     block_reduce_store<3>(sum, partials, P);
 }
 template <int EXTRA>
-__global__ __launch_bounds__(kBlock, 2) void k_round0_dot29(FactorPtrs fp, uint64_t q, FieldParams P, uint64_t *__restrict__ partials) {
-    round0_dot29_body<EXTRA>(fp, q, P, partials);
+__global__ __launch_bounds__(kBlock, 2) void k_round0_dot29(FactorPtrs fp, uint64_t q, FieldParams P, uint64_t *__restrict__ partials, uint64_t rev = 0) {
+    round0_dot29_body<EXTRA>(fp, q, P, partials, rev);
 }
 template <int EXTRA>
-__global__ __launch_bounds__(kBlock, 2) void k_round0_dot29_b(BatchOf<RoundSlot> b, uint64_t q, FieldParams P) {
+__global__ __launch_bounds__(kBlock, 2) void k_round0_dot29_b(BatchOf<RoundSlot> b, uint64_t q, FieldParams P, uint64_t rev = 0) {
     const RoundSlot &a = b.a[blockIdx.y];
     const FactorPtrs fp = factor_ptrs_of(a.fp);
-    round0_dot29_body<EXTRA>(fp, q, P, a.partials);
+    round0_dot29_body<EXTRA>(fp, q, P, a.partials, rev);
 }
 
 extern __shared__ __attribute__((aligned(1024))) uint8_t glds_ring[];
@@ -490,8 +495,9 @@
     uint32_t my_lds;
     uint32_t lane, voff, own;
     uint64_t r0, rs, K;
+    uint64_t rm;
 };
-ZK_D GldsWave glds_wave(uint64_t q, uint32_t nblk, uint32_t bytes_per_wave = 8192) {
+ZK_D GldsWave glds_wave(uint64_t q, uint32_t nblk, uint32_t bytes_per_wave = 8192, uint64_t rev = 0) {
     GldsWave w;
     w.lane = threadIdx.x & 63;
     const uint32_t wave = __builtin_amdgcn_readfirstlane(threadIdx.x >> 6);
@@ -503,6 +509,7 @@
     w.r0 = (uint64_t)blockIdx.x * (kBlock / 64) + wave;
     w.rs = (uint64_t)nblk * (kBlock / 64);
     w.K = w.r0 < runs ? (runs - w.r0 + w.rs - 1) / w.rs : 0;
+    w.rm = rev >> 6;
     return w;
 }
 
@@ -519,9 +526,9 @@
     for (int i = 0; i < 17; ++i) c[i] = 0;
 }
 template <int EXTRA>
-ZK_D void round0_glds_body(const FactorPtrs &fp, uint64_t q, const FieldParams &P, uint64_t *__restrict__ partials) {
+ZK_D void round0_glds_body(const FactorPtrs &fp, uint64_t q, const FieldParams &P, uint64_t *__restrict__ partials, uint64_t rev = 0) {
     constexpr int NU = 2 + EXTRA;
-    const GldsWave w = glds_wave(q, gridDim.x, NU * 4096);
+    const GldsWave w = glds_wave(q, gridDim.x, NU * 4096, rev);
     const uint64_t hi_off = q * 32;
     uint64_t c0[17], c1[17], cL[17];
 #pragma unroll
@@ -531,13 +538,13 @@
     if (w.K) {
 #pragma unroll
         for (int f = 0; f < NU; ++f) {
-            const uint64_t a = (uint64_t)(uintptr_t)fp.in[f] + w.r0 * 2048;
+            const uint64_t a = (uint64_t)(uintptr_t)fp.in[f] + sweep_index(w.r0, w.rm) * 2048;
             glds_rows2(a, a + hi_off, w.voff, w.my_lds + f * 4096);
         }
         int since = 0, lazy = 0;
         for (uint64_t k = 0; k < w.K; ++k) {
             const bool last = k + 1 == w.K;
-            const uint64_t next = (w.r0 + (k + 1) * w.rs) * 2048;
+            const uint64_t next = sweep_index(w.r0 + (k + 1) * w.rs, w.rm) * 2048;
             uint32_t la0[9], la1[9], ld0[9];
             round0_glds_wait<NU, 0>(last);
             {
@@ -593,19 +600,19 @@
     block_reduce_store<3>(sum, partials, P);
 }
 template <int EXTRA>
-__global__ __launch_bounds__(kBlock, 2) void k_round0_glds(FactorPtrs fp, uint64_t q, FieldParams P, uint64_t *__restrict__ partials) {
-    round0_glds_body<EXTRA>(fp, q, P, partials);
+__global__ __launch_bounds__(kBlock, 2) void k_round0_glds(FactorPtrs fp, uint64_t q, FieldParams P, uint64_t *__restrict__ partials, uint64_t rev = 0) {
+    round0_glds_body<EXTRA>(fp, q, P, partials, rev);
 }
 template <int EXTRA>
-__global__ __launch_bounds__(kBlock, 2) void k_round0_glds_b(BatchOf<RoundSlot> b, uint64_t q, FieldParams P) {
+__global__ __launch_bounds__(kBlock, 2) void k_round0_glds_b(BatchOf<RoundSlot> b, uint64_t q, FieldParams P, uint64_t rev = 0) {
     const RoundSlot &a = b.a[blockIdx.y];
     const FactorPtrs fp = factor_ptrs_of(a.fp);
-    round0_glds_body<EXTRA>(fp, q, P, a.partials);
+    round0_glds_body<EXTRA>(fp, q, P, a.partials, rev);
 }
 
 template <int F, int K, int EXTRA, bool STORE_NT>
-ZK_D void fused_glds_unit(const GldsWave &w, const FactorPtrs &fp, uint64_t q, uint64_t run, bool last, const Mul29 &r, const FieldParams &P,
-                          Fe (&prod)[K + 1], WideAcc (&acc)[K + 1], Fe (&sum_b)[K + 1]) {
+ZK_D void fused_glds_unit(const GldsWave &w, const FactorPtrs &fp, uint64_t q, uint64_t run, uint64_t next_run, bool last, const Mul29 &r,
+                          const FieldParams &P, Fe (&prod)[K + 1], WideAcc (&acc)[K + 1], Fe (&sum_b)[K + 1]) {
     constexpr int D = K, NT = K + EXTRA;
     const Fe c0 = glds_elem(w.my, w.own), c1 = glds_elem(w.my + 2048, w.own), c2 = glds_elem(w.my + 4096, w.own), c3 = glds_elem(w.my + 6144, w.own);
     asm volatile("s_waitcnt lgkmcnt(0)" ::: "memory");
@@ -614,7 +621,7 @@
         const uint64_t a = (uint64_t)(uintptr_t)fp.in[F + 1 < NT ? F + 1 : 0] + run * 2048;
         glds_rows4(a, a + rowb, a + 2 * rowb, a + 3 * rowb, w.voff, w.my_lds);
     } else if (!last) {
-        const uint64_t a = (uint64_t)(uintptr_t)fp.in[0] + (run + w.rs) * 2048;
+        const uint64_t a = (uint64_t)(uintptr_t)fp.in[0] + next_run * 2048;
         glds_rows4(a, a + rowb, a + 2 * rowb, a + 3 * rowb, w.voff, w.my_lds);
     }
     const Fe lo = fe_sub(c0, fe_mul29(fe_sub(c0, c2, P), r, P), P);
@@ -647,7 +654,7 @@
 }
 template <int K, int EXTRA, bool STORE_NT>
 ZK_D void fused_glds_body(const FactorPtrs &fp, uint64_t q, const FieldParams &P, const uint64_t *__restrict__ rptr, uint64_t *__restrict__ partials,
-                          const ClaimJob &cj) {
+                          const ClaimJob &cj, uint64_t rev = 0) {
     constexpr int NS = K + 1;
     uint32_t nblk = gridDim.x;
     if (cj.out) {
@@ -662,7 +669,7 @@
     }
     const Mul29 r = load_challenge29(rptr);
     asm volatile("s_waitcnt vmcnt(0)" ::: "memory");
-    const GldsWave w = glds_wave(q, nblk);
+    const GldsWave w = glds_wave(q, nblk, 8192, rev);
     Fe prod[NS], sum[NS], sum_b[NS];
     WideAcc acc[NS];
 #pragma unroll
@@ -673,17 +680,17 @@
     }
     if (w.K) {
         {
-            const uint64_t a = (uint64_t)(uintptr_t)fp.in[0] + w.r0 * 2048, rowb = q * 32;
+            const uint64_t a = (uint64_t)(uintptr_t)fp.in[0] + sweep_index(w.r0, w.rm) * 2048, rowb = q * 32;
             glds_rows4(a, a + rowb, a + 2 * rowb, a + 3 * rowb, w.voff, w.my_lds);
         }
         wait_vm<0>();
         for (uint64_t k = 0; k < w.K; ++k) {
-            const uint64_t run = w.r0 + k * w.rs;
+            const uint64_t run = sweep_index(w.r0 + k * w.rs, w.rm), next_run = sweep_index(w.r0 + (k + 1) * w.rs, w.rm);
             const bool last = k + 1 == w.K;
-            fused_glds_unit<0, K, EXTRA, STORE_NT>(w, fp, q, run, last, r, P, prod, acc, sum_b);
-            fused_glds_unit<1, K, EXTRA, STORE_NT>(w, fp, q, run, last, r, P, prod, acc, sum_b);
-            if constexpr (K + EXTRA > 2) fused_glds_unit<2, K, EXTRA, STORE_NT>(w, fp, q, run, last, r, P, prod, acc, sum_b);
-            if constexpr (K + EXTRA > 3) fused_glds_unit<3, K, EXTRA, STORE_NT>(w, fp, q, run, last, r, P, prod, acc, sum_b);
+            fused_glds_unit<0, K, EXTRA, STORE_NT>(w, fp, q, run, next_run, last, r, P, prod, acc, sum_b);
+            fused_glds_unit<1, K, EXTRA, STORE_NT>(w, fp, q, run, next_run, last, r, P, prod, acc, sum_b);
+            if constexpr (K + EXTRA > 2) fused_glds_unit<2, K, EXTRA, STORE_NT>(w, fp, q, run, next_run, last, r, P, prod, acc, sum_b);
+            if constexpr (K + EXTRA > 3) fused_glds_unit<3, K, EXTRA, STORE_NT>(w, fp, q, run, next_run, last, r, P, prod, acc, sum_b);
         }
 #pragma unroll
         for (int t = 0; t < NS; ++t)
@@ -698,14 +705,14 @@
 }
 template <int K, int EXTRA, bool STORE_NT>
 __global__ __launch_bounds__(kBlock, 2) void k_round_fused_glds(FactorPtrs fp, uint64_t q, FieldParams P, const uint64_t *__restrict__ rptr,
-                                                                 uint64_t *__restrict__ partials, ClaimJob cj) {
-    fused_glds_body<K, EXTRA, STORE_NT>(fp, q, P, rptr, partials, cj);
+                                                                 uint64_t *__restrict__ partials, ClaimJob cj, uint64_t rev = 0) {
+    fused_glds_body<K, EXTRA, STORE_NT>(fp, q, P, rptr, partials, cj, rev);
 }
 template <int K, int EXTRA, bool STORE_NT>
-__global__ __launch_bounds__(kBlock, 2) void k_round_fused_glds_b(BatchOf<RoundSlot> b, uint64_t q, FieldParams P) {
+__global__ __launch_bounds__(kBlock, 2) void k_round_fused_glds_b(BatchOf<RoundSlot> b, uint64_t q, FieldParams P, uint64_t rev = 0) {
     const RoundSlot &a = b.a[blockIdx.y];
     const FactorPtrs fp = factor_ptrs_of(a.fp);
-    fused_glds_body<K, EXTRA, STORE_NT>(fp, q, P, a.rptr, a.partials, a.cj);
+    fused_glds_body<K, EXTRA, STORE_NT>(fp, q, P, a.rptr, a.partials, a.cj, rev);
 }
 
 template <int K, int D, int EXTRA>
diff --git a/zk_amd/csrc/rounds.hip b/zk_amd/csrc/rounds.hip
--- a/zk_amd/csrc/rounds.hip
+++ b/zk_amd/csrc/rounds.hip
@@ -31,6 +31,11 @@
     return v;
 }
 static bool glds_takes(uint64_t q, uint64_t min_pairs) { return glds_rounds() && (q & 63) == 0 && q >= 64 && q >= glds_min_pairs(min_pairs); }
+bool sweep_alternates(uint64_t bytes, uint64_t prev_bytes) {
+    static const bool on = env_u64("ZK_SWEEP_ALT", 1, 0, 1) != 0;
+    static const uint64_t min_bytes = env_u64("ZK_SWEEP_ALT_MIN_BYTES", (uint64_t)1792 << 20, 0, (uint64_t)1 << 50);
+    return on && bytes + prev_bytes > min_bytes;
+}
 static uint64_t quad_max_pairs() {
     static const uint64_t v = env_u64("ZK_QUAD_MAX_PAIRS", (uint64_t)1 << 15, 0, (uint64_t)1 << 40);
     return v;
@@ -77,16 +82,20 @@
 constexpr uint32_t kd_shape(int K, int D, bool FUSED, int EXTRA, bool SKIP1, bool LEAD) {
     return (uint32_t)K | ((uint32_t)D << 4) | ((uint32_t)FUSED << 8) | ((uint32_t)EXTRA << 9) | ((uint32_t)SKIP1 << 10) | ((uint32_t)LEAD << 11);
 }
+static inline uint64_t rev_kd(const RoundLaunchCtx &lc, uint64_t q) { return sweep_mask(q, kBlock, lc.reverse); }
+static inline uint64_t rev_glds(const RoundLaunchCtx &lc, uint64_t q) { return sweep_mask(q, 64, lc.reverse); }
 template <int K, int D, bool FUSED, int EXTRA = 0, bool SKIP1 = false, bool LEAD = false>
 static void go_kd(const RoundLaunchCtx &lc, const FactorPtrs &fp, uint64_t q, const uint64_t *d_r, uint32_t grid, const ClaimJob &cj = {}) {
     const FieldParams *P = lc.P;
     hipStream_t st = lc.stream;
     uint64_t *part = lc.d_partials;
-    auto single = [=]() {
-        k_round_kd<K, D, FUSED, EXTRA, SKIP1, LEAD><<<grid, kBlock, 0, st>>>(fp, q, *P, d_r, part, cj);
-        return hipGetLastError();
-    };
-    if (batch_record(BK_ROUND_KD, kd_shape(K, D, FUSED, EXTRA, SKIP1, LEAD), grid, kBlock, 0, q, 0, 0, 0, RoundSlot{factor_ptrs4(fp), d_r, part, cj}, single))
+    const uint64_t rev = rev_kd(lc, q);
+    auto single = [=]() {
+        k_round_kd<K, D, FUSED, EXTRA, SKIP1, LEAD><<<grid, kBlock, 0, st>>>(fp, q, *P, d_r, part, cj, rev);
+        return hipGetLastError();
+    };
+    if (batch_record(BK_ROUND_KD, kd_shape(K, D, FUSED, EXTRA, SKIP1, LEAD), grid, kBlock, 0, q, rev, 0, 0, RoundSlot{factor_ptrs4(fp), d_r, part, cj},
+                     single))
         return;
     (void)single();
 }
@@ -95,11 +104,12 @@
     const FieldParams *P = lc.P;
     hipStream_t st = lc.stream;
     uint64_t *part = lc.d_partials;
-    auto single = [=]() {
-        k_round0_dot29<EXTRA><<<grid, kBlock, 0, st>>>(fp, q, *P, part);
-        return hipGetLastError();
-    };
-    if (batch_record(BK_ROUND0_DOT29, (uint32_t)EXTRA, grid, kBlock, 0, q, 0, 0, 0, RoundSlot{factor_ptrs4(fp), nullptr, part, ClaimJob{}}, single)) return;
+    const uint64_t rev = rev_kd(lc, q);
+    auto single = [=]() {
+        k_round0_dot29<EXTRA><<<grid, kBlock, 0, st>>>(fp, q, *P, part, rev);
+        return hipGetLastError();
+    };
+    if (batch_record(BK_ROUND0_DOT29, (uint32_t)EXTRA, grid, kBlock, 0, q, rev, 0, 0, RoundSlot{factor_ptrs4(fp), nullptr, part, ClaimJob{}}, single)) return;
     (void)single();
 }
 
@@ -110,11 +120,12 @@
     hipStream_t st = lc.stream;
     uint64_t *part = lc.d_partials;
     constexpr uint32_t lds = EXTRA ? kGldsRing3Bytes : kGldsRingBytes;
-    auto single = [=]() {
-        k_round0_glds<EXTRA><<<grid, kBlock, lds, st>>>(fp, q, *P, part);
-        return hipGetLastError();
-    };
-    if (batch_record(BK_ROUND0_DOT29, kShapeGlds | (uint32_t)EXTRA, grid, kBlock, lds, q, 0, 0, 0, RoundSlot{factor_ptrs4(fp), nullptr, part, ClaimJob{}}, single)) return;
+    const uint64_t rev = rev_glds(lc, q);
+    auto single = [=]() {
+        k_round0_glds<EXTRA><<<grid, kBlock, lds, st>>>(fp, q, *P, part, rev);
+        return hipGetLastError();
+    };
+    if (batch_record(BK_ROUND0_DOT29, kShapeGlds | (uint32_t)EXTRA, grid, kBlock, lds, q, rev, 0, 0, RoundSlot{factor_ptrs4(fp), nullptr, part, ClaimJob{}}, single)) return;
     (void)single();
 }
 template <int K, int EXTRA>
@@ -123,12 +134,13 @@
     hipStream_t st = lc.stream;
     uint64_t *part = lc.d_partials;
     const bool nt = q >= glds_nt_min_pairs();
-    auto single = [=]() {
-        if (nt) k_round_fused_glds<K, EXTRA, true><<<grid, kBlock, kGldsRingBytes, st>>>(fp, q, *P, d_r, part, cj);
-        else k_round_fused_glds<K, EXTRA, false><<<grid, kBlock, kGldsRingBytes, st>>>(fp, q, *P, d_r, part, cj);
-        return hipGetLastError();
-    };
-    if (batch_record(BK_ROUND_KD, kd_shape(K, K, true, EXTRA, true, true) | kShapeGlds | (nt ? kShapeGldsNt : 0u), grid, kBlock, kGldsRingBytes, q, 0, 0, 0,
+    const uint64_t rev = rev_glds(lc, q);
+    auto single = [=]() {
+        if (nt) k_round_fused_glds<K, EXTRA, true><<<grid, kBlock, kGldsRingBytes, st>>>(fp, q, *P, d_r, part, cj, rev);
+        else k_round_fused_glds<K, EXTRA, false><<<grid, kBlock, kGldsRingBytes, st>>>(fp, q, *P, d_r, part, cj, rev);
+        return hipGetLastError();
+    };
+    if (batch_record(BK_ROUND_KD, kd_shape(K, K, true, EXTRA, true, true) | kShapeGlds | (nt ? kShapeGldsNt : 0u), grid, kBlock, kGldsRingBytes, q, rev, 0, 0,
                      RoundSlot{factor_ptrs4(fp), d_r, part, cj}, single))
         return;
     (void)single();
@@ -301,18 +313,18 @@
     BatchOf<RoundSlot> slots;
     batch_gather(r, idx, slots);
     const dim3 grid(r0.grid, (uint32_t)r.n);
-    const uint64_t q = r0.s[0];
+    const uint64_t q = r0.s[0], rev = r0.s[1];
     const FieldParams &P = *r.P;
 #define ZK_KD_B(K, D, F, E, S, L)                                                                  \
     case kd_shape(K, D, F, E, S, L):                                                               \
-        k_round_kd_b<K, D, F, E, S, L><<<grid, kBlock, 0, r.stream>>>(slots, q, P);               \
+        k_round_kd_b<K, D, F, E, S, L><<<grid, kBlock, 0, r.stream>>>(slots, q, P, rev);          \
         break;
     if (r0.kernel == BK_ROUND_KD && (r0.shape & kShapeGlds)) {
         const uint32_t base = r0.shape & ~(kShapeGlds | kShapeGldsNt);
         const bool nt = (r0.shape & kShapeGldsNt) != 0;
         if (base == kd_shape(3, 3, true, 0, true, true)) {
-            if (nt) k_round_fused_glds_b<3, 0, true><<<grid, kBlock, kGldsRingBytes, r.stream>>>(slots, q, P);
-            else k_round_fused_glds_b<3, 0, false><<<grid, kBlock, kGldsRingBytes, r.stream>>>(slots, q, P);
+            if (nt) k_round_fused_glds_b<3, 0, true><<<grid, kBlock, kGldsRingBytes, r.stream>>>(slots, q, P, rev);
+            else k_round_fused_glds_b<3, 0, false><<<grid, kBlock, kGldsRingBytes, r.stream>>>(slots, q, P, rev);
         } else {
             return kLaunchUnsupported;
         }
@@ -328,12 +340,12 @@
             default: return kLaunchUnsupported;
         }
     } else if (r0.kernel == BK_ROUND0_DOT29 && r0.shape == kShapeGlds) {
-        k_round0_glds_b<0><<<grid, kBlock, kGldsRingBytes, r.stream>>>(slots, q, P);
+        k_round0_glds_b<0><<<grid, kBlock, kGldsRingBytes, r.stream>>>(slots, q, P, rev);
     } else if (r0.kernel == BK_ROUND0_DOT29 && r0.shape == (kShapeGlds | 1u)) {
-        k_round0_glds_b<1><<<grid, kBlock, kGldsRing3Bytes, r.stream>>>(slots, q, P);
+        k_round0_glds_b<1><<<grid, kBlock, kGldsRing3Bytes, r.stream>>>(slots, q, P, rev);
     } else if (r0.kernel == BK_ROUND0_DOT29) {
         if (r0.shape != 0) return kLaunchUnsupported;
-        k_round0_dot29_b<0><<<grid, kBlock, 0, r.stream>>>(slots, q, P);
+        k_round0_dot29_b<0><<<grid, kBlock, 0, r.stream>>>(slots, q, P, rev);
     } else if (r0.kernel == BK_ROUND_QUAD) {
         if (r0.shape == (2u | (2u << 4))) k_round_quad_b<2, 2, 0><<<grid, kBlock, 0, r.stream>>>(slots, q, P);
         else if (r0.shape == (3u | (3u << 4))) k_round_quad_b<3, 3, 0><<<grid, kBlock, 0, r.stream>>>(slots, q, P);
diff --git a/zk_amd/csrc/sweep_index.hpp b/zk_amd/csrc/sweep_index.hpp
--- /dev/null
+++ b/zk_amd/csrc/sweep_index.hpp
@@ -0,0 +1,18 @@
+#pragma once
+#include <cstdint>
+
+#if defined(__HIPCC__) || defined(__CUDACC__)
+#define ZK_SWEEP_HD __host__ __device__ inline
+#else
+#define ZK_SWEEP_HD inline
+#endif
+
+namespace zk {
+
+ZK_SWEEP_HD uint64_t sweep_mask(uint64_t q, uint64_t tile, bool reversed) {
+    const bool pow2 = q != 0 && (q & (q - 1)) == 0 && tile != 0 && (tile & (tile - 1)) == 0;
+    return (reversed && pow2 && q >= tile) ? (q - 1) & ~(tile - 1) : 0;
+}
+ZK_SWEEP_HD uint64_t sweep_index(uint64_t j, uint64_t mask) { return j ^ mask; }
+
+}
```
